# orchidas/DiffGFDN

Measured on AMD Instinct MI355X. Metric: RIR-frames/sec, higher is better.
Workload: dtype f32

## Files before the change

### diffgfdn_amd/_lib.py

```python
import ctypes
import os
from ctypes import c_char_p, c_double, c_float, c_int, c_size_t, c_void_p

_HERE = os.path.dirname(os.path.abspath(__file__))
LIB_PATH = os.path.join(_HERE, "lib", "libdiffgfdn_hip.so")
ABI_VERSION = 8

_P = c_void_p

SIGNATURES = {
    "gfdn_abi_version": (c_int, []),
    "gfdn_zprep": (c_int, [_P, c_int, _P, _P, _P]),
    "gfdn_ortho_fwd": (c_int, [_P, c_int, c_int, _P, _P, _P]),
    "gfdn_ortho_bwd": (c_int, [_P, c_int, c_int, _P, _P, _P, _P, _P]),
    "gfdn_coupled_feedback_fwd": (c_int, [_P, _P, c_int, c_int, c_int, _P, _P, _P]),
    "gfdn_coupled_feedback_bwd": (c_int, [_P, _P, c_int, c_int, c_int, _P, _P, _P, _P]),
    "gfdn_solve_fwd": (c_int, [_P, _P, c_int, c_int, c_int, _P, _P, _P, _P, c_int, _P, _P]),
    "gfdn_solve_bwd_work_bytes": (c_size_t, [c_int, c_int]),
    "gfdn_solve_bwd": (c_int, [_P, _P, c_int, c_int, c_int, _P, _P, _P, _P, c_int, _P, _P, _P, _P, _P, _P, _P]),
    "gfdn_solve_precise_fwd": (c_int, [_P, _P, c_int, c_int, c_int, _P, _P, _P, _P, c_int, _P, _P]),
    "gfdn_solve_precise_bwd": (c_int, [_P, _P, c_int, c_int, c_int, _P, _P, _P, _P, c_int, _P, _P, _P, _P, _P, _P, _P]),
    "gfdn_solve_absorb_fwd": (c_int, [_P, _P, c_int, c_int, c_int, _P, _P, _P, _P, _P, c_int, _P, _P]),
    "gfdn_solve_absorb_bwd": (c_int, [_P, _P, c_int, c_int, c_int, _P, _P, _P, _P, _P, c_int, _P, _P, _P, _P, _P, _P, _P]),
    "gfdn_solve_phi_fwd": (c_int, [_P, _P, c_int, c_int, c_int, _P, _P, _P, _P, _P, _P, _P]),
    "gfdn_solve_phi_bwd_work_bytes": (c_size_t, [c_int, c_int]),
    "gfdn_solve_phi_bwd": (c_int, [_P, _P, c_int, c_int, c_int, _P, _P, _P, _P, _P, _P, _P, _P, _P, _P, _P, _P, _P]),
    "gfdn_solve_phi_absorb_fwd": (c_int, [_P, _P, c_int, c_int, c_int, _P, _P, _P, _P, _P, _P, _P, _P]),
    "gfdn_solve_phi_absorb_bwd": (c_int, [_P, _P, c_int, c_int, c_int, _P, _P, _P, _P, _P, _P, _P, _P, _P, _P, _P, _P, _P,
                                          _P]),
    "gfdn_svf_coefficients": (c_int, [_P, _P, ctypes.c_double, c_int, c_int, _P, _P, _P]),
    "gfdn_sos_response": (c_int, [_P, c_int, c_int, _P, c_int, _P, _P]),
    "gfdn_sos_compose_fwd": (c_int, [_P, c_int, c_int, c_int, _P, c_int, _P, _P, c_int, _P, _P]),
    "gfdn_sos_compose_bwd_chunks": (c_int, [c_int, c_int, _P, _P]),
    "gfdn_sos_compose_bwd": (c_int, [_P, c_int, c_int, c_int, _P, c_int, _P, _P, _P, _P, _P]),
    "gfdn_compose_fwd": (c_int, [_P, c_int, c_int, c_int, _P, _P, c_int, _P, c_int, _P, _P, _P, c_int, _P, _P]),
    "gfdn_compose_bwd_work_bytes": (c_size_t, [c_int, c_int, c_int, c_int]),
    "gfdn_compose_bwd": (c_int, [_P, c_int, c_int, c_int, _P, _P, c_int, _P, _P, c_int, _P, _P, _P, _P, _P]),
    "gfdn_compose_banded_fwd": (c_int, [_P, c_int, c_int, c_int, c_int, _P, _P, c_int, _P, c_int, _P, _P, c_int, _P, c_int, _P, _P]),
    "gfdn_compose_banded_bwd_work_bytes": (c_size_t, [c_int, c_int, c_int, c_int, c_int]),
    "gfdn_compose_banded_bwd": (c_int, [_P, c_int, c_int, c_int, c_int, _P, _P, c_int, _P, c_int, _P, c_int, _P, _P, _P, _P, _P]),
    "gfdn_compose_sh_fwd": (c_int, [_P, c_int, c_int, c_int, _P, _P, c_int, _P, _P, _P]),
    "gfdn_compose_sh_bwd_work_bytes": (c_size_t, [c_int, c_int, c_int]),
    "gfdn_compose_sh_bwd": (c_int, [_P, c_int, c_int, c_int, _P, _P, c_int, _P, _P, _P, _P, _P, _P, _P]),
    "gfdn_spectral_stats_work_bytes": (c_size_t, [c_int, c_int]),
    "gfdn_spectral_stats": (c_int, [_P, c_int, c_int, c_int, c_float, _P, _P, _P, _P, _P]),
    "gfdn_colorless_terms": (c_int, [_P, c_int, _P, c_int, c_float, c_float, c_float, _P, _P, _P]),
    "gfdn_colorless_terms_banded": (c_int, [_P, c_int, c_int, _P, c_int, c_float, c_float, c_float, _P, _P, _P]),
    "gfdn_weighted_sums_banded": (c_int, [_P, c_int, _P, _P, c_float, _P, c_float, c_int, c_int, _P, _P]),
    "gfdn_mlp_gains_banded_fwd": (c_int, [_P, _P, _P, _P, c_int, c_int, c_int, c_int, c_int, c_int, c_float, c_float, _P, _P, _P, _P]),
    "gfdn_mlp_gains_banded_bwd": (c_int, [_P, _P, _P, _P, c_int, c_int, c_int, c_int, c_int, c_int, c_float, c_float, _P, _P, _P, _P, _P, _P, _P]),
    "gfdn_mlp_gains_banded_bwd_parts": (c_int, [_P, _P, _P, _P, c_int, c_int, c_int, c_int, c_int, c_int, c_float, c_float, _P, _P, _P, _P, c_int, _P, _P, _P]),
    "gfdn_mlp_gains_banded_bwd_parts_scaled": (c_int, [_P, _P, _P, _P, c_int, c_int, c_int, c_int, c_int, c_int, c_float, c_float,
                                                       _P, _P, _P, _P, c_int, _P, _P, _P, _P]),
    "gfdn_tf_gain_chunks": (c_int, [c_int]),
    "gfdn_mlp_bwd_takes_parts": (c_int, [c_int, c_int, c_int, c_int, c_int]),
    "gfdn_mlp_bands_sizes": (c_int, [c_int, c_int, c_int, _P, _P, c_int, _P]),
    "gfdn_mlp_gains_bands_fwd": (c_int, [_P, _P, _P, _P, c_int, c_int, c_int, _P, _P, c_int, c_float, c_float, _P, _P, _P, _P]),
    "gfdn_mlp_gains_bands_bwd": (c_int, [_P, _P, _P, _P, c_int, c_int, c_int, _P, _P, c_int, c_float, c_float, _P, _P, _P, _P,
                                         c_int, _P, _P, _P, _P]),
    "gfdn_subfdn_normalize_work_bytes": (c_size_t, [c_int]),
    "gfdn_subfdn_normalize": (c_int, [_P, _P, c_int, c_int, c_int, _P, _P, _P, _P, _P, _P, _P]),
    "gfdn_subfdn_colorless_work_bytes": (c_size_t, [c_int, c_int]),
    "gfdn_subfdn_colorless_fwd": (c_int, [_P, _P, c_int, c_int, c_int, _P, _P, _P, _P, c_int, _P, _P, _P, _P, _P]),
    "gfdn_spectral_stats_binmajor": (c_int, [_P, c_int, c_int, _P, c_int, c_float, _P, _P, _P, _P]),
    "gfdn_subfdn_colorless_bwd": (c_int, [_P, _P, c_int, c_int, c_int, _P, _P, _P, _P, _P, _P, _P, _P, _P, _P, _P, _P]),
    "gfdn_tf_coefs_fwd": (c_int, [_P, _P, _P, _P, c_int, c_int, _P, _P]),
    "gfdn_tf_coefs_fwd2": (c_int, [_P, _P, _P, _P, _P, _P, _P, _P, c_int, c_int, _P]),
    "gfdn_tf_ortho_coefs": (c_int, [_P, _P, _P, _P, c_int, c_int, _P, _P, _P, _P, _P]),
    "gfdn_tf_coefs_bwd": (c_int, [_P, _P, _P, _P, _P, _P, _P, _P, c_int, c_int, _P, _P, _P, _P, _P]),
    "gfdn_tf_param_grads": (c_int, [_P, _P, _P, c_int, _P, _P, _P, _P, _P, c_int, c_int, _P, _P, _P, _P, _P, _P, _P]),
    "gfdn_tf_rows_sum": (c_int, [_P, c_int, c_int, _P, _P]),
    "gfdn_tf_parts": (c_int, [c_int, c_int]),
    "gfdn_tf_work_bytes": (c_size_t, [c_int]),
    "gfdn_tf_gpart_bytes": (c_size_t, [c_int]),
    "gfdn_tf_eval": (c_int, [_P, _P, c_int, c_int, c_int, _P, _P, _P, _P, _P]),
    "gfdn_tf_energy": (c_int, [_P, _P, c_int, c_int, c_int, _P, _P, _P, _P, _P, _P, _P, c_int, c_double, _P]),
    "gfdn_tf_energy_gains": (c_int, [_P, _P, c_int, c_int, c_int, _P, _P, _P, _P, _P, _P, _P, c_int, c_double, _P, _P, c_int, c_int,
                                     _P]),
    "gfdn_tf_colorless": (c_int, [_P, _P, c_int, c_int, c_int, _P, _P, _P, c_int, c_float, _P, _P, _P, c_double, _P]),
    "gfdn_tf_compose_fwd": (c_int, [_P, _P, c_int, c_int, c_int, c_int, _P, _P, _P, _P, c_int, _P, c_int, _P, _P, c_int, _P, c_int, _P, _P,
                                    _P]),
    "gfdn_tf_compose_parts": (c_int, [c_int]),
    "gfdn_tf_compose_bwd_work_bytes": (c_size_t, [c_int, c_int, c_int]),
    "gfdn_tf_compose_bwd": (c_int, [_P, _P, c_int, c_int, c_int, c_int, _P, _P, _P, _P, _P, c_int, _P, c_int, _P, c_int, _P, _P,
                                    c_int, _P]),
    "gfdn_tf_tail": (c_int, [_P, _P, _P, c_int, _P, _P, _P, _P, c_int, c_int, _P, _P, _P, _P, _P, _P, _P, _P, _P, _P, _P, _P,
                             _P, c_int, c_int, c_int, c_float, c_float, c_float, _P, _P, _P, _P, _P]),
    "gfdn_irfft_odd_pairs_bwd_tslots3": (c_int, [_P, c_int, _P, _P, _P, c_int, c_int, _P, c_int, _P, _P]),
    "gfdn_irfft_odd_pairs_fwd_scaled": (c_int, [_P, c_int, _P, c_int, c_int, _P, _P, c_int, _P, c_int, _P]),
    "gfdn_edc_lin_one_max_len": (c_int, []),
    "gfdn_edc_lin_one": (c_int, [_P, c_int, _P, _P, c_int, _P, c_int, c_int, c_int, c_int, c_int, _P, _P, c_int, _P, _P,
                                 c_int, c_float, c_float, _P, _P, c_int, _P, c_int, c_int, _P]),
    "gfdn_lin_merge_slots": (c_int, [_P, _P, _P, c_int, c_int, c_int, _P, _P, c_int, _P]),
    "gfdn_f64_fft_work_bytes": (c_size_t, [c_int, c_int]),
    "gfdn_irfft_odd_f64_length": (c_int, [c_int]),
    "gfdn_rfft_pow2_f64": (c_int, [_P, c_int, c_int, c_int, c_int, _P, c_int, _P, _P]),
    "gfdn_irfft_odd_f64_plan": (c_int, [c_int, _P, _P, _P]),
    "gfdn_irfft_odd_f64": (c_int, [_P, c_int, _P, c_int, c_int, _P, _P, _P, c_int, _P, _P]),
    "gfdn_lin_gamma_win": (c_int, [_P, c_int, _P, c_int, c_int, c_int, c_int, c_int, c_int, _P, _P, _P, c_int, _P, _P, c_int,
                                   _P]),
    "gfdn_tf_gain_grad_work_bytes": (c_size_t, [c_int, c_int, c_int, c_int]),
    "gfdn_tf_gain_grad": (c_int, [c_int, c_int, c_int, c_int, _P, _P, c_int, _P, c_int, _P, _P, _P]),
    "gfdn_tf8_coefs": (c_int, [_P, _P, _P, _P, _P, _P, _P, _P, c_int, c_int, _P]),
    "gfdn_tf8_parts": (c_int, [c_int]),
    "gfdn_tf8_part_bytes": (c_size_t, [c_int, c_int]),
    "gfdn_tf8_energy": (c_int, [_P, c_int, c_int, c_int, _P, _P, _P, _P, _P, _P, _P, c_double, _P]),
    "gfdn_tf8_tsave": (c_int, [_P, c_int, c_int, c_int, c_int, _P, _P, _P, _P, _P, _P, _P, c_int, _P, _P, _P, _P]),
    "gfdn_tf8_colorless": (c_int, [_P, c_int, c_int, c_int, _P, _P, _P, _P, c_int, c_float, _P, _P, _P, c_double, _P]),
    "gfdn_tf8_compose_bwd": (c_int, [_P, c_int, c_int, c_int, c_int, _P, _P, _P, _P, _P, c_int, _P, c_int, _P, c_int, _P,
                                     _P, _P, _P]),
    "gfdn_tf8_param_grads_work_bytes": (c_size_t, [c_int]),
    "gfdn_tf8_param_grads": (c_int, [_P, _P, _P, c_int, _P, _P, _P, c_int, _P, _P, c_int, c_int, _P, _P, _P, _P, _P, _P, _P,
                                     _P]),
    "gfdn_tfp_parts": (c_int, []),
    "gfdn_tfp_forward": (c_int, [c_int, c_int, c_int, c_int, _P, _P, _P, c_int, _P, _P, c_int, _P, _P]),
    "gfdn_tfp_energy": (c_int, [_P, _P, c_int, c_int, c_int, c_int, _P, _P, _P, _P, _P, _P, _P, c_int, c_int, _P]),
    "gfdn_tfp_colorless": (c_int, [_P, _P, c_int, c_int, c_int, c_int, _P, _P, c_int, c_float, c_int, _P, _P, c_int, _P, _P, _P,
                                   _P, _P]),
    "gfdn_tfp_compose_bwd": (c_int, [c_int, c_int, c_int, c_int, _P, c_int, _P, _P, c_int, _P, c_int, _P, _P, _P, c_int, c_int,
                                     _P, c_int, _P, c_int, _P, _P, _P]),
    "gfdn_tf8_tail": (c_int, [_P, _P, _P, c_int, _P, _P, c_int, _P, _P, c_int, c_int, _P, _P, _P, _P, _P, _P, _P, _P, _P, _P, _P,
                              _P, _P, _P, c_int, c_int, c_int, c_float, c_float, c_float, _P, _P, _P, _P]),
    "gfdn_tf9_coefs": (c_int, [_P, _P, _P, c_int, c_int, _P, _P]),
    "gfdn_tf9_rec_grads_work_bytes": (c_size_t, [c_int]),
    "gfdn_tf9_rec_grads": (c_int, [_P, _P, _P, _P, _P, c_int, c_int, _P, _P, _P, _P, _P]),
    "gfdn_tfp_ratio_fwd": (c_int, [_P, _P, c_int, c_int, c_int, _P, _P, _P]),
    "gfdn_tfp_ratio_bwd": (c_int, [c_int, c_int, c_int, c_int, _P, _P, c_int, _P, _P, c_int, _P, c_int, _P, c_int, _P, _P, _P]),
    "gfdn_ortho_bwd_add": (c_int, [_P, c_int, c_int, _P, _P, _P, _P, _P, _P]),
    "gfdn_exp_contract_mfma": (c_int, [_P, c_int, _P, _P, c_int, _P, _P]),
    "gfdn_weighted_sums": (c_int, [_P, c_int, _P, _P, c_float, _P, c_float, c_int, _P, _P]),
    "gfdn_normalize_io": (c_int, [_P, _P, _P, c_int, c_int, _P]),
    "gfdn_bluestein_table_bytes": (c_size_t, [c_int]),
    "gfdn_bluestein_table_init": (c_int, [c_int, _P]),
    "gfdn_bluestein_work_bytes": (c_size_t, [c_int, c_int]),
    "gfdn_irfft_odd_fwd": (c_int, [_P, c_int, _P, c_int, c_int, _P, c_int, _P, _P]),
    "gfdn_irfft_odd_bwd": (c_int, [_P, c_int, _P, _P, c_int, c_int, _P, c_int, _P, _P]),
    "gfdn_irfft_odd_slot_order": (c_int, [c_int, _P, _P]),
    "gfdn_irfft_odd_slots_fwd": (c_int, [_P, c_int, _P, c_int, c_int, _P, c_int, _P, _P]),
    "gfdn_irfft_odd_slots_bwd": (c_int, [_P, c_int, _P, _P, c_int, c_int, _P, c_int, _P, _P]),
    "gfdn_irfft_odd_pairs_fwd": (c_int, [_P, c_int, _P, c_int, c_int, _P, c_int, _P, _P]),
    "gfdn_irfft_odd_pairs_compose_fwd": (c_int, [_P, c_int, _P, c_int, _P, _P, c_int, _P, _P, c_int, c_int, c_int, c_int, _P,
                                                 _P, c_int, _P, c_int, _P]),
    "gfdn_irfft_odd_pairs_bwd": (c_int, [_P, c_int, _P, _P, c_int, c_int, _P, c_int, _P, _P]),
    "gfdn_irfft_odd_pairs_gains_parts": (c_int, [c_int]),
    "gfdn_irfft_odd_pairs_gains_bwd": (c_int, [_P, c_int, _P, _P, c_int, c_int, _P, c_int, _P, c_int, _P, c_int, c_int, c_int, _P,
                                               _P, c_int, _P]),
    "gfdn_stft_power_pairs": (c_int, [_P, c_int, c_int, c_int, c_int, _P, _P, _P]),
    "gfdn_stft_power_pairs_bwd": (c_int, [_P, c_int, c_int, c_int, c_int, _P, _P, _P, _P]),
    "gfdn_stft_power_pairs_bwd_phase": (c_int, [_P, c_int, c_int, c_int, c_int, _P, _P, _P, c_int, _P]),
    "gfdn_edc_loss_pairs": (c_int, [_P, c_int, c_int, c_int, c_int, _P, _P, _P, c_float, c_float, _P, _P, _P, _P]),
    "gfdn_irfft_odd_stages": (c_int, [_P, c_int, _P, _P, c_int, c_int, _P, c_int, _P, c_int, c_int, c_int, _P]),
    "gfdn_irfft_pow2_work_bytes": (c_size_t, [c_int, c_int]),
    "gfdn_irfft_pow2_fwd": (c_int, [c_int, _P, c_int, c_int, _P, c_int, _P, _P]),
    "gfdn_irfft_pow2_fwd_band": (c_int, [c_int, _P, c_int, c_int, c_int, _P, c_int, c_int, _P, _P]),
    "gfdn_irfft_pow2_bwd": (c_int, [c_int, _P, c_int, c_int, _P, c_int, _P, _P]),
    "gfdn_rownorm_fwd": (c_int, [_P, c_int, c_int, c_float, _P, _P]),
    "gfdn_rownorm_bwd": (c_int, [_P, c_int, c_int, c_float, _P, _P, _P]),
    "gfdn_irfft_pow2_bwd_window": (c_int, [c_int, _P, c_int, c_int, c_int, c_int, _P, c_int, _P, _P]),
    "gfdn_edc_mixed_work_bytes": (c_size_t, [c_int, c_int, c_int]),
    "gfdn_edc_loss_model_mixed": (c_int, [_P, c_int, c_int, c_int, _P, c_int, c_int, c_int, _P, c_int, _P, c_int, _P,
                                          c_float, c_float, _P, _P, _P, _P]),
    "gfdn_group_sums_fwd": (c_int, [_P, c_int, c_int, c_int, _P, _P, _P]),
    "gfdn_group_sums_bwd": (c_int, [_P, c_int, c_int, c_int, _P, _P, _P, _P, _P, _P]),
    "gfdn_dirlin_tiles": (c_int, [c_int]),
    "gfdn_dirlin_line_tiles": (c_int, [c_int]),
    "gfdn_dirlin_lines_fwd": (c_int, [_P, c_int, c_int, _P, _P, _P, c_int, _P]),
    "gfdn_dirlin_lines_bwd": (c_int, [_P, c_int, c_int, _P, _P, _P, c_int, _P, _P, _P, _P]),
    "gfdn_dirlin_combine": (c_int, [_P, c_int, c_int, c_int, _P, c_int, c_int, c_int, _P, c_int, _P]),
    "gfdn_dirlin_gamma_dots": (c_int, [_P, c_int, c_int, _P, c_int, c_int, _P, c_int, c_int, c_int, _P, c_int, _P, _P, _P]),
    "gfdn_edc_loss_model_mixed_stages": (c_int, [_P, c_int, c_int, c_int, _P, c_int, c_int, c_int, _P, c_int, _P, c_int, _P,
                                                 c_float, c_float, _P, _P, _P, c_int, _P]),
    "gfdn_rfft_pow2": (c_int, [c_int, _P, c_int, c_int, c_int, _P, c_int, _P, _P]),
    "gfdn_sh_to_directional": (c_int, [_P, c_int, c_int, c_int, c_int, _P, _P, c_int, _P]),
    "gfdn_stft_nframes": (c_int, [c_int, c_int]),
    "gfdn_stft_power": (c_int, [_P, c_int, c_int, c_int, c_int, _P, _P, _P]),
    "gfdn_stft_power_bwd": (c_int, [_P, c_int, c_int, c_int, c_int, _P, _P, _P]),
    "gfdn_edr_work_bytes": (c_size_t, [c_int, c_int]),
    "gfdn_edr_target": (c_int, [_P, c_int, c_int, c_int, _P, _P, _P]),
    "gfdn_edr_loss": (c_int, [_P, _P, _P, _P, _P, c_int, c_int, c_int, c_float, c_int, _P, _P, _P]),
    "gfdn_edc_work_bytes": (c_size_t, [c_int]),
    "gfdn_edc_target": (c_int, [_P, c_int, c_int, c_int, c_int, _P, _P, _P]),
    "gfdn_mlp_param_count": (c_size_t, [c_int, c_int, c_int, c_int]),
    "gfdn_mlp_bwd_work_bytes": (c_size_t, [c_int, c_int, c_int, c_int, c_int]),
    "gfdn_mlp_gains_fwd": (c_int, [_P, _P, _P, _P, c_int, c_int, c_int, c_int, c_int, c_float, c_float, _P, _P, _P, _P]),
    "gfdn_mlp_gains_bwd": (c_int, [_P, _P, _P, _P, c_int, c_int, c_int, c_int, c_int, c_float, c_float, _P, _P, _P, _P, _P, _P, _P]),
    "gfdn_pick_rows": (c_int, [_P, _P, _P, c_int, _P]),
    "gfdn_adam_step": (c_int, [_P, _P, _P, _P, _P, _P, _P, c_int, c_float, c_float, c_float, _P]),
    "gfdn_adam_step_counted": (c_int, [_P, _P, _P, _P, _P, _P, _P, c_int, c_float, c_float, c_float, _P, _P]),
    "gfdn_adam_step_mirrored": (c_int, [_P, _P, _P, _P, _P, _P, _P, _P, c_int, c_float, c_float, c_float, _P, _P]),
    "gfdn_edc_loss": (c_int, [_P, c_int, c_int, c_int, c_int, _P, _P, _P, c_float, c_float, _P, _P, _P, _P]),
    "gfdn_edc_loss_model": (c_int, [_P, c_int, c_int, c_int, c_int, _P, c_int, _P, c_int, _P, c_float, c_float, _P, _P, _P, _P]),
    "gfdn_draw_mask": (c_int, [ctypes.c_ulonglong, _P, c_int, c_float, _P, _P]),
    "gfdn_lin_gain_chunks": (c_int, [c_int]),
    "gfdn_lin_combine_fwd": (c_int, [_P, c_int, _P, _P, c_int, c_int, _P, c_int, c_int, c_int, c_int, _P, c_int, c_int, _P]),
    "gfdn_lin_gamma": (c_int, [_P, _P, c_int, c_int, _P, c_int, c_int, c_int, c_int, _P, c_int, c_int, _P, _P, c_int, _P]),
    "gfdn_lin_gamma_dots_tiles": (c_int, [c_int]),
    "gfdn_lin_gamma_dots": (c_int, [_P, c_int, _P, c_int, c_int, c_int, c_int, _P, c_int, _P, c_int, _P, _P, c_int, _P, c_int,
                                    c_int, c_int, _P, _P, _P]),
    "gfdn_stft_pairs_spectrum": (c_int, [_P, c_int, c_int, c_int, c_int, _P, c_int, _P]),
    "gfdn_stft_pairs_spectrum_bwd": (c_int, [_P, c_int, c_int, c_int, _P, _P, c_int, c_int, c_int, _P, _P]),
    "gfdn_edr_lin_parts": (c_int, [c_int]),
    "gfdn_edr_lin_loss": (c_int, [_P, _P, _P, _P, c_int, c_int, c_int, _P, _P, c_int, c_int, c_float, c_int, _P, _P, _P, c_int,
                                  c_int, c_int, _P]),
    "gfdn_edr_lin_gsum": (c_int, [_P, _P, _P, _P, c_int, c_int, c_int, _P, c_int, c_int, _P, _P]),
    "gfdn_edr_lin_loss_gsum": (c_int, [_P, _P, _P, _P, c_int, c_int, c_int, _P, _P, c_int, c_int, c_float, _P, c_int, _P,
                                       c_int, c_int, _P, c_int, c_int, _P]),
    "gfdn_edr_lin_band_parts": (c_int, [c_int]),
    "gfdn_edc_loss_pairs_lin": (c_int, [_P, c_int, _P, _P, c_int, _P, c_int, c_int, c_int, c_int, c_int, c_int, _P, _P, c_int,
                                        _P, _P, c_int, c_float, c_float, _P, _P, c_int, _P, _P, _P]),
    "gfdn_irfft_odd_time_slots": (c_int, [c_int, _P]),
    "gfdn_irfft_odd_pairs_bwd_tslots": (c_int, [_P, c_int, _P, c_int, c_int, _P, c_int, _P, _P]),
    "gfdn_lin_gain_dots": (c_int, [_P, _P, c_int, c_int, _P, c_int, c_int, c_int, c_int, c_int, c_int, _P, c_int, _P]),
    "gfdn_edc_loss_banded": (c_int, [_P, c_int, c_int, c_int, c_int, _P, _P, c_int, _P, _P, c_int, c_int, c_float, c_float,
                                     _P, _P, _P, _P]),
    "gfdn_edc_loss_pairs_banded": (c_int, [_P, c_int, c_int, c_int, c_int, _P, _P, c_int, _P, _P, c_int, c_int, c_float,
                                           c_float, _P, _P, _P, _P]),
    "gfdn_draw_mask_banded": (c_int, [ctypes.c_ulonglong, _P, _P, c_int, c_int, c_int, c_float, _P, _P]),
    "gfdn_render_mix": (c_int, [_P, c_int, _P, _P, _P, c_int, c_int, c_int, c_int, _P, c_int, _P]),
}

_lib = None


def load():
    global _lib
    if _lib is not None:
        return _lib
    if not os.path.exists(LIB_PATH):
        raise RuntimeError(
            f"diffgfdn_amd: HIP library not built ({LIB_PATH}); run `make -C diffgfdn_amd/csrc` "
            "or `python -c 'import __graft_entry__ as g; g.build()'`. There is no CPU fallback.")
    import torch
    lib = ctypes.CDLL(LIB_PATH)
    for name, (res, args) in SIGNATURES.items():
        fn = getattr(lib, name)
        fn.restype = res
        fn.argtypes = args
    ver = lib.gfdn_abi_version()
# ... 11 lines not shown
```

### diffgfdn_amd/bankstep.py

```python
import contextlib
from typing import Dict, NamedTuple, Optional

import torch

from . import hip_ops as ops
from .functional import FrequencyGrid
from .losses import shard_loss_scales


_Plan = NamedTuple('_Plan', [
    ('nb', int), ('G', int), ('n', int), ('K', int), ('Ku', int), ('Btot', int), ('Bper', int), ('win', int), ('start', int),
    ('length', int),
    ('order', Optional[tuple]), ('sot', Optional[torch.Tensor]), ('tfp', Optional[tuple]),
    ('item_len', Optional[torch.Tensor]), ('band_len', Optional[torch.Tensor]),
    ('train', bool), ('normalize_first', bool), ('opt_step', bool), ('reduced', bool), ('piped', bool),
    ('big', bool), ('late', bool), ('late8', bool),
    ('lin', bool), ('spec', bool), ('pairs', bool), ('fold', bool),
    ('gfold', bool), ('parts_in_mlp', bool), ('net_first', bool), ('edc_one', bool), ('late_colorless', bool),
    ('use_tail', bool), ('use_tail8', bool), ('keep_records', bool)])


class _Step:
    scale = Hg = Ts = Dinv8 = ework = Xsub = rgain0 = rgain = xhat = rstd = H = Tq = tau = eye = xd = None
    ev_ts = ev_gam = gH = gsig = gsig_b = g_edc = gam_edr = parts = grg = None
# ... 73 lines not shown
            Q, QQ, cs = self._records()
            q, qq = ops.ortho_fwd(bank._blocks().detach(), True, True)
            Q.copy_(q)
            QQ.copy_(qq)
            cs.copy_(bank.output_gains.data.view(-1))
            self._rec_valid, self._rec_versions = True, self._versions()
            return
        ops.tf_ortho_coefs(bank._blocks().detach(), bank.inv_gamma, bank.input_gains.data.view(-1),
                           bank.output_gains.data.view(-1), out=self._records())
        self._rec_valid, self._rec_versions = True, self._versions()

    def ensure_records(self):
        if self._rec is not None and not self.records_ok():
            self.prime_records()

    linear_transforms = True
    spectral_edr = True
    edc_one_launch = True
    scale_late = True
    fused_tail = True
    transform_polys = True
    edr_one_launch = True
    edr_receiver_runs = 0

    def _edr_runs(self, nbands: int, B: int) -> int:
        if self.edr_receiver_runs > 0:
            return min(self.edr_receiver_runs, B)
        return 2 if B >= 4 else 1
    tiled_spectra = True

    def _eye_rows(self, nb: int, G: int, device) -> torch.Tensor:
        key = (nb, G, str(device))
        if getattr(self, '_eye_cache', None) is None or self._eye_cache[0] != key:
            self._eye_cache = (key, torch.eye(G, dtype=torch.float32, device=device).repeat(nb, 1).contiguous())
        return self._eye_cache[1]

    def _plan(self, data: Dict, maskw, how, reduced: bool, piped: bool) -> "_Plan":
        tr = self.tr
        normalize_first, train, opt_step = how
        bank, nb = tr.net, tr.num_bands
        G, n = bank.num_groups, bank.num_delay_lines_per_group
        z, rows = data['z_values'], data['row_index']
        Btot = rows.numel()
        if Btot % nb:
            raise ValueError("the batch must hold the same number of receivers for every band")
        Bper, K, win = Btot // nb, z.shape[-1], tr.stft_win
        side2 = tr._stream('_side2') is not None
        gridK = FrequencyGrid.of(z)
        order = ops.irfft_slot_order(K, z.device) if (tr.use_slot_order and 'dataset' in data) else None
        lin = (self.linear_transforms and not piped and ops.lin_supported(Bper, G)
               and hasattr(data.get('dataset'), 'direct_time'))
        start, length = tr._decay_window(K)
        item_len, band_len = tr._item_windows(K, Bper, z.device)
        if item_len is not None and (maskw is None or maskw.ndim != 2):
            raise ValueError("bands with different EDC windows: pass the (bands, window) weight rows of "
                             "BandBankTrainer._band_mask_rows as maskw")
        pairs = order is not None and tr.use_pairs and win == 4096
        big = n > 4
        if big and (gridK.logr is not None):
            raise NotImplementedError("blocks of more than four lines: the explicit step takes grids on the unit circle "
                                      "(set BandBankTrainer.use_fused = False to step this bank through the per-bin "
                                      "elimination kernels under autograd)")
        tail_ok = self.fused_tail and train and opt_step and not reduced and not piped and side2
        use_tail = tail_ok and not big
        late = self.scale_late and lin and order is not None and normalize_first and not big and side2
        tfp = None
        if big and self.transform_polys and lin and order is not None and gridK.rfft_nfft and side2 and normalize_first:
            T_seq = ops.tfp_plan(bank.delays, n, gridK.rfft_nfft)
            sob = ops.tfp_slot_of_bin(K, z.device)
            if T_seq is not None and sob is not None:
                tfp = (gridK.rfft_nfft, sob, T_seq)
        late8 = tfp is not None
        use_tail8 = tail_ok and late8
        spec = (lin and self.spectral_edr and pairs and ops.spec_supported(Bper, G)
                and hasattr(data['dataset'], 'direct_stft'))
        Hh, n_hidden = bank._mlp_cfg[0], bank._mlp_cfg[1]
        parts_in_mlp = ops.mlp_bwd_takes_parts(bank._freq_pi.numel(), Hh, n_hidden, G, Bper)
        if piped and (not train or reduced or not opt_step or not side2):
            raise ValueError("a pipelined step is a single-process training step with its optimiser update")
        if big:
            keep_records = use_tail8 and self.records_ok()
        else:
            keep_records = self.records_ok() and (use_tail or not train)
        return _Plan(
            nb=nb, G=G, n=n, K=K, Ku=(K + 1) // 2 if K % 2 == 1 else K, Btot=Btot, Bper=Bper, win=win, start=start,
            length=length, order=order, tfp=tfp, item_len=item_len, band_len=band_len,
            sot=ops.irfft_slot_of_time(K, z.device) if (lin and train and order is not None) else None,
            train=train, normalize_first=normalize_first, opt_step=opt_step, reduced=reduced, piped=piped, big=big, lin=lin,
            pairs=pairs, spec=spec, late=late, late8=late8, use_tail=use_tail, use_tail8=use_tail8, keep_records=keep_records,
            parts_in_mlp=parts_in_mlp,
            gfold=(late or late8) and not piped and spec and train and parts_in_mlp,
            fold=pairs and K == 65537 and Bper % 2 == 0 and G <= 4 and not lin,
            late_colorless=big or spec,
            edc_one=self.edc_one_launch and ops.edc_lin_one_supported(length, G),
            net_first=bool(getattr(bank, 'mixed_networks', False)))

    def _begin(self, p: "_Plan", data: Dict, maskw, inv: float, calls: Dict) -> "_Step":
        tr = self.tr
        bank, z = tr.net, data['z_values']
        if p.lin:
            zu, direct = (data['dataset'].slot_grid(*p.order) if p.order is not None else z[:p.Ku]), None
        elif p.order is not None:
            zu, direct = data['dataset'].slot_ordered(*p.order)
        else:
            zu, direct = z[:p.Ku], data['target_early_response'][:, :p.Ku]
        return _Step(
            **calls, data=data, rows=data['row_index'], maskw=maskw, inv=inv, keep=self._keep,
            main=torch.cuda.current_stream(), side=tr._stream('_side'), side2=tr._stream('_side2'),
            M=bank._blocks().detach(), b=bank.input_gains.data.view(-1), c=bank.output_gains.data.view(-1),
            delays=bank.delays, ig=bank.inv_gamma, w=bank.output_scalars_w.detach(), gridK=FrequencyGrid.of(z), zu=zu,
            direct=direct, inv_world=shard_loss_scales(tr.world_size, 1, 1.0)['colorless'],
            T_edr=data['edr_target'][1], sum_abs=data['edr_target'][2], T_edc=data['edc_target'][1],
            ev={k: torch.cuda.Event() for k in ('start', 'g', 'h', 'mlp', 'mask', 'norm', 'x', 'edc', 'side', 'grg', 'mlpb')})

    def _gain_network(self, st: "_Step", out=None):
        bank = self.tr.net
        Hh, n_hidden, _, lo, hi = bank._mlp_cfg
        return ops.mlp_gains_fwd(st.data['norm_listener_position'], bank._freq_pi, st.w, Hh, n_hidden, bank.num_groups, lo, hi,
                                 st.rows, self.tr.num_bands, out=out)

    def _wait_gains(self, st: "_Step"):
        if st.pipe is None:
            st.main.wait_event(st.ev['mlp'])
        elif st.pipe.ready is not None:
            st.main.wait_event(st.pipe.ready)

    def _records_head(self, p: "_Plan", st: "_Step"):
        ev, keep, late_any = st.ev, st.keep, p.late or p.late8
        if not late_any:
            ev['start'].record()
        st.c_head = st.c
        if p.big:
            if p.keep_records:
                st.Q, st.QQ, st.c_head = self._records()
            else:
                st.Q, st.QQ = ops.ortho_fwd(st.M, True, True)
                if p.late8:
                    st.c_head = st.c.detach().clone()
                    keep.append(st.c_head)
            st.coef, st.coef_sub = ops.tf8_coefs(st.QQ, st.ig, st.b, st.c, A1=st.M)
        else:
            if not p.keep_records:
                ops.tf_ortho_coefs(st.M, st.ig, st.b, st.c, out=self._records())
            st.Q, st.QQ, st.coef, st.coef_sub = self._records()
        self._rec_valid = False
        if late_any:
            ev['start'].record()
        st.gridU = FrequencyGrid.of(st.zu)
        st.filt = self.tr._filter_on(p.Ku, p.order)
        gridK, gridU = st.gridK, st.gridU
        if p.late:
            st.Hg, st.Ts = ops.tf_compose_fwd(gridU.turns, gridU.logr, st.coef, st.delays, p.n,
                                              self._eye_rows(p.nb, p.G, st.rows.device), None, None, st.filt, None, p.nb,
                                              save_T=True, want_H=True)
        if p.late8:
            st.Ts, _, st.Hg, st.Dinv8 = ops.tf8_tsave(gridK.turns[:p.Ku], st.coef, st.delays, p.n, st.c_head, None, p.nb, p.G,
                                                      quad=False, filt=st.filt, want_H=True, hslot=p.tfp[1])
            keep.append(st.Dinv8)
        if p.normalize_first and not late_any:
            if p.big:
                _, st.scale = ops.tf8_energy(gridK.turns, st.coef_sub, st.delays, p.n, st.b, st.c, dturn=gridK.dturn)
            else:
                _, st.scale = ops.tf_energy(gridK.turns, gridK.logr, st.coef_sub, st.delays, p.n, st.b, st.c,
                                            want_energy=False, dturn=gridK.dturn)
        if not late_any:
            ev['norm'].record()

    def _side_head(self, p: "_Plan", st: "_Step"):
        ev, keep, gridK, pipe = st.ev, st.keep, st.gridK, st.pipe
        energy = (gridK.turns, gridK.logr, st.coef_sub, st.delays, p.n, st.b, st.c)
        with st.on_side2():
            if pipe is None or pipe.first:
                torch.cuda.current_stream().wait_event(ev['start'])
            if p.gfold and p.big:
                st.rgain0, st.xhat, st.rstd = self._gain_network(st)
                keep.append(st.rgain0)
            if p.late:
                if p.gfold:
                    if p.net_first:
                        st.rgain0, st.xhat, st.rstd = self._gain_network(st)
                    st.ework = ops.tf_energy(*energy, phase=1, dturn=gridK.dturn)
                    if not p.net_first:
                        st.rgain0, st.xhat, st.rstd = self._gain_network(st)
                    keep.append(st.rgain0)
                    _, st.scale, st.rgain = ops.tf_energy(*energy, want_energy=False, work=st.ework, phase=2,
                                                          dturn=gridK.dturn, gains=st.rgain0, G=p.G)
                else:
                    _, st.scale = ops.tf_energy(*energy, want_energy=False, dturn=gridK.dturn)
                ev['norm'].record()
            elif p.late8:
                nblk8 = p.nb * p.G
                st.Xsub = ops.tfp_forward(st.coef_sub, st.delays, st.c, p.n, p.tfp[0], p.tfp[2])
                if p.gfold:
                    _, st.scale, st.rgain = ops.tfp_energy(st.Xsub[:nblk8], st.Xsub[nblk8:], p.n, st.b, st.c, gains=st.rgain0,
                                                           G=p.G)
                else:
                    _, st.scale = ops.tfp_energy(st.Xsub[:nblk8], st.Xsub[nblk8:], p.n, st.b, st.c)
                ev['norm'].record()
                keep.append(st.Xsub)
            if p.gfold:
                ev['mlp'].record()
            elif pipe is None:
                st.rgain, st.xhat, st.rstd = self._gain_network(st)
                ev['mlp'].record()
            else:
                st.rgain, st.xhat, st.rstd = pipe.cur
            if st.mask_draw is not None:
                st.mask_draw()
            ev['mask'].record()

    def _group_signals(self, p: "_Plan", st: "_Step"):
        gridU, K = st.gridU, p.K
        st.eye = self._eye_rows(p.nb, p.G, st.rows.device)
        st.xd = st.data['dataset'].direct_time(self.tr.subband_filter_freq_resp, K)
        if p.late8:
            pass
        elif p.big:
            st.Ts, _, st.Hg, st.Dinv8 = ops.tf8_tsave(gridU.turns, st.coef, st.delays, p.n, st.c, st.scale, p.nb, p.G,
                                                      quad=False, filt=st.filt, want_H=True)
            st.keep.append(st.Dinv8)
            st.ev_ts = torch.cuda.Event()
            st.ev_ts.record()
        elif not p.late:
            st.Hg, st.Ts = ops.tf_compose_fwd(gridU.turns, gridU.logr, st.coef, st.delays, p.n, st.eye, st.scale, None,
                                              st.filt, None, p.nb, save_T=True, want_H=True)
        if p.gfold:
            st.tau = ops.irfft_odd_fwd(st.Hg, K, slots=True, pairs=True)
        elif p.late or p.late8:
            st.tau = ops.irfft_odd_fwd(st.Hg, K, slots=True, pairs=True, oscale=st.scale,
                                       before_last=lambda: st.main.wait_event(st.ev['norm']))
        else:
            st.tau = ops.irfft_odd_fwd(st.Hg, K, slots=p.order is not None, pairs=p.order is not None)
        st.H = st.Hg
        st.keep.extend((st.tau, st.xd))

    def _stored_output_stage(self, p: "_Plan", st: "_Step"):
        gridU = st.gridU
        if not p.fold:
            self._wait_gains(st)
        if p.big:
            st.Ts, Tq8 = ops.tf8_tsave(gridU.turns, st.coef, st.delays, p.n, st.c, st.scale, p.nb, p.G, quad=True)
            st.ev_ts = torch.cuda.Event()
            st.ev_ts.record()
            if p.fold:
                st.H = Tq8
            else:
                Hs = torch.einsum('qbg,qgk->qbk', st.rgain.reshape(p.nb, p.Bper, p.G).to(torch.complex64),
                                  st.Ts.reshape(p.nb, p.G, -1))
                Hs = Hs + st.direct[st.rows].reshape(p.nb, p.Bper, -1)[..., :st.Ts.shape[1]]
                if st.filt is not None:
                    Hs = Hs * st.filt.reshape(p.nb, 1, -1)
                st.H = Hs.reshape(p.Btot, -1).contiguous()
        else:
            st.H, st.Ts = ops.tf_compose_fwd(gridU.turns, gridU.logr, st.coef, st.delays, p.n, st.rgain, st.scale, st.direct,
                                             st.filt, st.rows, p.nb, save_T=True, want_H=not p.fold)
        if p.fold:
            st.Tq, st.H = st.H, None

    def _colorless(self, p: "_Plan", st: "_Step"):
        cfg, gridK, weight = self.tr.config, st.gridK, self.tr.config.spectral_loss_weight * st.inv_world
        with st.on_side2():
            if not p.late and not p.late8:
                torch.cuda.current_stream().wait_event(st.ev['norm'])
            if p.late8:
                nblk8 = p.nb * p.G
                grec_sub, loss_g = ops.tfp_colorless(st.Xsub[:nblk8], st.Xsub[nblk8:], p.tfp[0], p.n, st.delays, st.scale,
                                                     cfg.use_asym_spectral_loss, weight, T=p.tfp[2])
            elif p.big:
                torch.cuda.current_stream().wait_event(st.ev_ts)
                grec_sub, loss_g = ops.tf8_colorless(gridK.turns, st.coef_sub, st.delays, p.n, st.c, st.scale,
                                                     cfg.use_asym_spectral_loss, weight, dturn=gridK.dturn)
            else:
                grec_sub, loss_g = ops.tf_colorless(gridK.turns, gridK.logr, st.coef_sub, st.delays, p.n, st.scale,
                                                    cfg.use_asym_spectral_loss, weight, dturn=gridK.dturn)
            st.out3, st.gQ = ops.colorless_terms(loss_g, st.Q, cfg.spectral_loss_weight, cfg.sparsity_loss_weight,
                                                 st.inv_world, want_grad=p.train, nbands=p.nb)
            st.ev['side'].record()
        st.grec_sub = grec_sub
        st.keep.extend((grec_sub, loss_g, st.out3, st.gQ))

    def _receiver_signals(self, p: "_Plan", st: "_Step") -> torch.Tensor:
        if p.lin:
            self._wait_gains(st)
            return ops.lin_combine_fwd(st.xd, st.rows, st.tau, st.rgain, p.nb, p.K, p.order is not None, p.pairs)
        if p.fold:
            self._wait_gains(st)
            x2, h0 = ops.irfft_odd_pairs_compose_fwd(st.direct, st.rows, st.Tq, st.rgain, st.filt, p.K, p.nb)
            st.keep.extend((h0, st.Tq))
            return x2
        if p.pairs:
            return ops.irfft_odd_fwd(st.H, p.K, slots=True, pairs=True)
        return ops.irfft_odd_fwd(st.H, p.K, slots=p.order is not None)

    def _decay_stored(self, p: "_Plan", st: "_Step"):
        cfg, keep, ev, main = self.tr.config, st.keep, st.ev, st.main
        K, Btot, win, train = p.K, p.Btot, p.win, p.train
        x = self._receiver_signals(p, st)
        ev['x'].record()
        if p.pairs:
            P = ops.stft_power_pairs(x, Btot, win)
            g_edr = None
        else:
            g_edr = torch.empty_like(x) if train else None
            P = ops.stft_power(x, win, zero_buf=g_edr)
        with st.on_side2():
            torch.cuda.current_stream().wait_event(ev['x'])
            if p.pairs:
                li_edc, g_edc = ops.edc_loss_pairs(x, Btot, p.start, p.length, st.T_edc, st.maskw, st.inv, cfg.edc_loss_weight,
                                                   train, rows=st.rows, item_len=p.item_len, items_per_band=p.Bper)
            else:
                li_edc, g_edc = ops.edc_loss(x, p.start, p.length, st.T_edc, st.maskw, st.inv, cfg.edc_loss_weight, train,
                                             rows=st.rows, item_len=p.item_len, items_per_band=p.Bper)
            ev['edc'].record()
        li_edr = ops.edr_loss(P, st.T_edr, st.sum_abs, None, cfg.edr_loss_weight, train, rows=st.rows, defer=True)
        keep.extend((x, P, g_edr, li_edc, g_edc, li_edr))
        gH = None
        if train:
            if p.pairs:
                g = ops.stft_power_pairs_bwd(x, Btot, win, P, phase=0)
                main.wait_event(ev['edc'])
                ops.stft_power_pairs_bwd(x, Btot, win, P, base=g_edc, out=g, phase=1)
                ev['g'].record()
                gH = (g, None) if p.lin else ops.irfft_odd_pairs_bwd(g, K, Btot)
                keep.append(g)
            else:
                g_edr = ops.stft_power_bwd(x, win, P, g_edr)
                main.wait_event(ev['edc'])
                ev['g'].record()
                if p.lin:
                    gH = (g_edc, g_edr)
                else:
                    gH = ops.irfft_odd_bwd(g_edc, K, (K + 1) // 2 if p.order is not None else st.H.shape[1], g_edr,
                                           slots=p.order is not None)
            keep.append(gH)
        else:
            main.wait_event(ev['edc'])
            ev['g'].record()
        st.li_edr, st.li_edc, st.gH = li_edr, li_edc, gH

    def _decay_spec(self, p: "_Plan", st: "_Step"):
        tr, cfg, keep, ev = self.tr, self.tr.config, st.keep, st.ev
        nb, G, K, win, train = p.nb, p.G, p.K, p.win, p.train
        rows, rgain, tau, ds, tiled = st.rows, st.rgain, st.tau, st.data['dataset'], self.tiled_spectra
        Sd = ds.direct_stft(tr.subband_filter_freq_resp, K, win, tiled=tiled)
        T_edr = ds.edr_target_tiled() if tiled else st.T_edr
        ev['x'].record()
        nch = 1 if p.edc_one else ops.lin_gamma_dots_tiles(K)
        parts = None
        if train:
            parts = torch.empty((p.Btot * G, nch + ops.edr_lin_parts(win // 2 + 1, fused=self.edr_one_launch)),
                                dtype=torch.float32, device=rows.device)
        Stau = ops.stft_pairs_spectrum(tau, nb * G, win, tiled=tiled)
        with st.on_side2():
            torch.cuda.current_stream().wait_event(ev['x'])
            edc_args = (st.xd, rows, tau, rgain, nb, K, p.start, p.length, st.T_edc, st.maskw, st.inv, cfg.edc_loss_weight,
                        train)
            if p.edc_one:
                li_edc, g_edc = ops.edc_lin_one(*edc_args, trows=rows, item_len=p.item_len, dots=parts, col=0)
                if train:
                    g_edc = (g_edc, ops.lin_gamma_win(g_edc, rgain, nb, K, p.start, p.length, band_win_len=p.band_len))
            else:
                li_edc, g_edc = ops.edc_loss_pairs_lin(*edc_args, trows=rows, item_len=p.item_len, fill_outside=False)
            ev['edc'].record()
        self._wait_gains(st)
        gP = Gs = None
        if train and self.edr_one_launch:
            li_edr, Gs = ops.edr_lin_loss_gsum(Sd, rows, Stau, rgain, nb, T_edr, st.sum_abs, cfg.edr_loss_weight, dots=parts,
                                               col0=nch, tiled=tiled, nsplit=self._edr_runs(nb, p.Bper))
        else:
            li_edr, gP = ops.edr_lin_loss(Sd, rows, Stau, rgain, nb, T_edr, st.sum_abs, cfg.edr_loss_weight, train,
                                          dots=parts, col0=nch, tiled=tiled)
        if not train:
            ev['g'].record()
        keep.extend((Sd, Stau, li_edc, g_edc, li_edr, gP, parts))
        st.li_edr, st.li_edc, st.gH = li_edr, li_edc, None
        if not train:
            st.main.wait_event(ev['edc'])
            return
        if Gs is None:
            Gs = ops.edr_lin_gsum(Sd, rows, Stau, rgain, nb, gP)
        gam_edr = ops.stft_pairs_spectrum_bwd(Gs, K, nb * G, win, tiled=tiled, split_parity=True)
        keep.extend((Gs, gam_edr))
        st.g_edc, st.gam_edr, st.parts = g_edc, gam_edr, parts

    def _report(self, p: "_Plan", st: "_Step"):
        cfg = self.tr.config
        s_ = ops.weighted_sums(st.li_edr, cfg.edr_loss_weight, st.li_edc, cfg.edc_loss_weight, st.sum_abs, st.rows, p.nb)
        st.sums, st.total = s_, ((s_[:, 0] + st.out3[:, 0]) if p.nb > 1 else (s_[0] + st.out3[0]))

    def _adjoint_signals(self, p: "_Plan", st: "_Step"):
        K, nb, keep = p.K, p.nb, st.keep
        if not p.lin:
            st.gH_rec, st.rg_rec = st.gH, st.rgain
            return
        tau_pairs = p.order is not None
        if p.spec:
            st.gsig, st.gsig_b = st.g_edc, None
            st.main.wait_event(st.ev['edc'])
            ge_a, ge_b = st.gam_edr if isinstance(st.gam_edr, tuple) else (st.gam_edr, None)
            if isinstance(st.gsig, tuple):
                gam = ops.lin_merge_slots(st.gsig[1], ge_a, ge_b, p.sot)
            else:
                gam = ops.lin_gamma_dots(st.gsig, st.rgain, nb, K, st.tau, st.parts, p.start, p.length, base=ge_a,
                                         slot_of_time=p.sot, band_win_len=p.band_len, base_b=ge_b)
            st.ev_gam = torch.cuda.Event()
            st.ev_gam.record()
        else:
            st.gsig, st.gsig_b = st.gH
            gam = ops.lin_gamma(st.gsig, st.rgain, nb, K, p.pairs, tau_pairs, gxb=st.gsig_b, slot_of_time=p.sot)
        if tau_pairs:
            gHg = ops.irfft_odd_pairs_bwd(gam, K, nb * p.G, tslots=p.sot is not None)
        else:
            gHg = ops.irfft_odd_bwd(gam, K, p.Ku, None, slots=False)
        keep.extend((gam, gHg, st.eye))
        st.gH_rec, st.rg_rec = gHg, st.eye

    def _records_pass(self, p: "_Plan", st: "_Step"):
        gridU = st.gridU
        if p.late8:
            st.grec = ops.tfp_compose_bwd(p.tfp[0], p.nb, p.G, p.n, st.delays, p.Ku, p.tfp[1], st.gH_rec, st.filt, st.Ts,
                                          st.Dinv8, tscale=st.scale, gain_fold=p.gfold, T=p.tfp[2])
        elif p.big:
            st.grec = ops.tf8_compose_bwd(gridU.turns, st.coef, st.delays, p.n, st.c, st.scale, st.rg_rec, st.gH_rec, st.filt,
                                          p.nb, saved=(st.Ts, st.Dinv8) if p.lin else None)
        else:
            st.grec = ops.tf_compose_bwd(gridU.turns, gridU.logr, st.coef, st.delays, p.n, st.rg_rec, st.gH_rec, st.Ts, st.filt,
                                         p.nb, partial=True, tscale=st.scale if p.late else None,
                                         gain_fold=p.gfold and p.late)

    def _side_backward(self, p: "_Plan", st: "_Step"):
        tr, ev, pipe = self.tr, st.ev, st.pipe
        bank, opt, nb, G = tr.net, tr.optimizer, p.nb, p.G
        Hh, n_hidden, _, lo, hi = bank._mlp_cfg
        with st.on_side2():
            cur = torch.cuda.current_stream()
            cur.wait_event(st.ev_gam if p.spec else ev['g'])
            self._report(p, st)
            if st.allreduce is not None:
                slots = opt.extra.view(3, nb)
                torch.stack((st.sums.reshape(nb, 3)[:, 1], st.sums.reshape(nb, 3)[:, 2], st.out3.reshape(nb, 3)[:, 0]),
                            out=slots)
            grg = None
            if p.lin:
                if p.spec:
                    cur.wait_event(st.ev_gam)
                    ggp = st.parts
                else:
                    ggp = ops.lin_gain_dots(st.gsig, st.tau, nb, p.Btot, G, p.K, p.pairs, p.order is not None, gxb=st.gsig_b)
                if not p.parts_in_mlp:
                    grg, ggp = ops.tf_rows_sum(ggp).view(p.Btot, G), None
            else:
                cur.wait_event(ev['grg'])
                if p.parts_in_mlp:
                    ggp = ops.tf_gain_grad(st.Ts, st.gH, G, st.filt, nb, partial=True)
                else:
                    grg, ggp = ops.tf_gain_grad(st.Ts, st.gH, G, st.filt, nb), None
            ops.mlp_gains_bwd(st.data['norm_listener_position'], bank._freq_pi, st.w, Hh, n_hidden, G, lo, hi,
                              st.rgain0 if p.gfold else st.rgain, st.xhat, st.rstd, grg, st.rows, nb, out=self.g_w,
                              ggains_parts=ggp, colscale=st.scale if p.gfold else None)
            st.keep.append(ggp)
            if pipe is not None:
                opt.step_range(*self.w_range, second=True)
                if st.tail is not None:
                    st.tail()
                self._gain_network(st, out=pipe.nxt)
                pipe.ready_next = torch.cuda.Event()
                pipe.ready_next.record()
            else:
                if p.use_tail or p.use_tail8:
                    opt.step_range(*self.w_range, second=True)
                ev['mlpb'].record()
                if st.tail is not None:
                    st.tail()
        st.grg = grg

    def _parameter_tail(self, p: "_Plan", st: "_Step"):
        tr, opt = self.tr, self.tr.optimizer
        rec = (st.QQ, st.ig, st.grec, st.grec_sub, st.b, st.c, st.M, st.gQ, st.Q, self.g_b, self.g_c)
        if p.use_tail8:
            ops.tf8_tail(*rec, self.g_M, opt, *self._off, *self._records())
        elif p.big:
            ops.tf8_param_grads(st.QQ, st.ig, st.grec, st.b, st.c, st.M, A1=st.M, part1=st.grec_sub, gQ=st.gQ, Q=st.Q,
                                gb=self.g_b, gc=self.g_c, gM=self.g_M)
        elif p.use_tail:
            ops.tf_tail(*rec, self.g_M.view(-1), opt, *self._off, *self._records())
        else:
            ops.tf_param_grads(st.QQ, st.ig, st.grec, st.b, st.c, st.M, A1=st.M, grec1=st.grec_sub, gQ=st.gQ, Q=st.Q,
                               gb=self.g_b, gc=self.g_c, gM=self.g_M)
        st.keep.extend((st.grg, st.grec))
        if p.piped:
            opt.step_range(0, self.w_range[0], second=False)
            torch.autograd.graph.increment_version(opt._params)
            return
        opt._packed = True
        if p.use_tail or p.use_tail8:
            opt._packed = False
            torch.autograd.graph.increment_version(opt._params)
            self._rec_valid, self._rec_versions = True, self._versions()
        elif p.opt_step and not p.reduced and st.side2 is not None:
            ev_pg = torch.cuda.Event()
            ev_pg.record()
            with st.on_side2():
                torch.cuda.current_stream().wait_event(ev_pg)
                self.finish(None)
        else:
            st.main.wait_event(st.ev['mlpb'])
            if p.opt_step:
                red = self.finish(st.allreduce)
                if red is not None:
                    st.sums, st.total = red

    def _losses(self, p: "_Plan", st: "_Step") -> Dict:
        col = (lambda t, i: t[:, i]) if p.nb > 1 else (lambda t, i: t[i])
        return {'edc_loss': col(st.sums, 2), 'edr_loss': col(st.sums, 1), 'spectral_loss': col(st.out3, 1),
                'sparsity_loss': col(st.out3, 2), '_total': st.total}

    def _end(self, p: "_Plan", st: "_Step") -> Dict:
        keep, pipe = st.keep, st.pipe
        keep.extend((st.sums, st.total))
        losses = self._losses(p, st)
        if pipe is None or pipe.last:
            for s_ in (st.side, st.side2):
                if s_ is not None:
                    st.main.wait_stream(s_)
        if pipe is not None:
            self._keep_prev = [] if pipe.last else list(keep)
            keep.clear()
            pipe.advance()
            return losses
        keep.clear()
        if not p.big and not p.train and not p.normalize_first:
            self._rec_valid, self._rec_versions = True, self._versions()
        return losses

    @torch.no_grad()
    def run(self, data: Dict, maskw: Optional[torch.Tensor], inv: float, normalize_first: bool, train: bool,
            allreduce=None, opt_step: bool = True, mask_draw=None, tail=None, pipe=None) -> Dict:
        p = self._plan(data, maskw, (normalize_first, train, opt_step), allreduce is not None, pipe is not None)
        st = self._begin(p, data, maskw, inv, dict(allreduce=allreduce, mask_draw=mask_draw, tail=tail, pipe=pipe))
        self._records_head(p, st)
        self._side_head(p, st)
        if p.lin:
            self._group_signals(p, st)
        else:
            self._stored_output_stage(p, st)
        st.keep.extend((st.coef_sub, st.ework, st.Q, st.QQ, st.coef, st.rgain, st.xhat, st.rstd, st.scale, st.H, st.Ts))
        if not p.late_colorless:
            self._colorless(p, st)
        st.ev['h'].record()
        if p.spec:
            self._decay_spec(p, st)
        else:
            self._decay_stored(p, st)
        if p.late_colorless:
            self._colorless(p, st)
        if not train:
            with st.on_side2():
                torch.cuda.current_stream().wait_event(st.ev['g'])
                self._report(p, st)
            return self._end(p, st)
        if (p.use_tail or p.use_tail8) and not torch.cuda.is_current_stream_capturing():
            self.tr.optimizer.sync_lr()
        st.ev['grg'].record()
        self._adjoint_signals(p, st)
        self._records_pass(p, st)
        self._side_backward(p, st)
        st.main.wait_event(st.ev['side'])
        self._parameter_tail(p, st)
        return self._end(p, st)

    def finish(self, allreduce):
        tr = self.tr
        nb = tr.num_bands
        red = None
        if allreduce is not None:
            allreduce()
        tr.optimizer.step()
        if allreduce is not None:
            slots = tr.optimizer.extra.view(3, nb)
            total = slots.sum(dim=0)
            sums = torch.stack((total, slots[0], slots[1]), dim=1)
# ... 33 lines not shown
```

### diffgfdn_amd/csrc/blocktf.hip

```cpp
#include "common.h"
#include "ortho_dev.h"

#define TF_MAXBLK 64
#define TF_REC 32
#define TF_MAXG 4
#define TF_MAX_PARTS 2048

__device__ __forceinline__ float2 tf_zpow(const double* __restrict__ turns, const double* __restrict__ logr,
                                          int k, float m) {
  double t = (double)m * turns[k];
  t -= rint(t);
  float s, c;
  sincospif(2.0f * (float)t, &s, &c);
  if (logr) {
    const float mag = (float)exp((double)m * logr[k]);
    c *= mag;
    s *= mag;
  }
  return make_float2(c, s);
}

__device__ __forceinline__ void tf_subsets(float2 (&e)[16]) {
  e[3] = cmul(e[1], e[2]);
  e[5] = cmul(e[1], e[4]);
// ... 676 lines not shown
extern "C" int gfdn_tf_energy_gains(const double* turns, const double* logr, int K, int nblk, int nper, const float* coef,
                                    const float* delays, float* b, float* c, float* energy, float* scale, void* work,
                                    int phase, double dturn, const float* gains, float* gains_scaled, int Bper, int G,
                                    void* stream) {
  if (!gains || !gains_scaled || Bper <= 0 || G <= 0 || nblk % G || !(phase & 2)) return GFDN_E_BADARG;
  return tf_energy_run(turns, logr, K, nblk, nper, coef, delays, b, c, energy, scale, work, phase, dturn, gains, gains_scaled, Bper,
                       G, stream);
}
static int tf_energy_run(const double* turns, const double* logr, int K, int nblk, int nper, const float* coef,
                         const float* delays, float* b, float* c, float* energy, float* scale, void* work, int phase,
                         double dturn, const float* gains, float* gains_scaled, int Bper, int G, void* stream) {
  int rc = tf_args_ok(turns, K, nblk, nper, coef, delays);
  if (rc) return rc;
  if (!work || (!b) != (!c) || !(phase & 3)) return GFDN_E_BADARG;
  TfArgs a{turns, logr, K, nblk, nper, coef, delays, nullptr};
  const int nparts = tf_parts_host(K, nblk);
  hipStream_t s = (hipStream_t)stream;
  if (phase & 1) {
    if (dturn != 0.0 && !logr)
      hipLaunchKernelGGL(k_tf_energy_runs, dim3(nparts), dim3(256), 0, s, a, dturn, (float*)work, tf_items(nblk));
    else
      hipLaunchKernelGGL(k_tf_energy, dim3(nparts), dim3(256), 0, s, a, (float*)work, tf_items(nblk));
    GFDN_LAUNCH_CHECK();
  }
  if (phase & 2) {
    hipLaunchKernelGGL(k_tf_energy_finish, dim3(nblk), dim3(256), 0, s, (const float*)work, nparts, K, nper, b, c,
                       energy, scale, gains, gains_scaled, Bper, G);
    GFDN_LAUNCH_CHECK();
  }
  return 0;
}

template <bool RUNS>
__global__ __launch_bounds__(256) void k_tf_colorless(TfArgs a, double dturn, int asym, float gscale,
                                                      float* __restrict__ gpart, int items) {
  extern __shared__ float tf_acc[];
  const int nblk = a.nblk;
  const bool live = (int)threadIdx.x < items;
  const int blk = live ? threadIdx.x % nblk : 0;
  const int krow = threadIdx.x / nblk, rows = items / nblk;
  float P[16], Q[16], m[4];
  tf_load(a.coef, a.delays, blk, a.nper, P, Q, m);
  const float sc = a.scale ? a.scale[blk] : 1.0f;
  const float invK = 1.0f / (float)a.K;
  float2 r0, r1, r2, r3;
  if (RUNS) {
    r0 = tf_rot(dturn, m[0]);
    r1 = tf_rot(dturn, m[1]);
    r2 = tf_rot(dturn, m[2]);
    r3 = tf_rot(dturn, m[3]);
  }
  float aP[16], aQ[16];
#pragma unroll
  for (int S = 0; S < 16; ++S) aP[S] = aQ[S] = 0.f;
  constexpr int RUN = RUNS ? TF_RUN : 1;
  const int nruns = (a.K + RUN - 1) / RUN;
#pragma unroll 1
  for (int run = blockIdx.x * rows + krow; live && run < nruns; run += gridDim.x * rows) {
    const int k0 = run * RUN;
    float2 e[16];
    e[1] = tf_zpow(a.turns, RUNS ? nullptr : a.logr, k0, m[0]);
    e[2] = tf_zpow(a.turns, RUNS ? nullptr : a.logr, k0, m[1]);
    e[4] = tf_zpow(a.turns, RUNS ? nullptr : a.logr, k0, m[2]);
    e[8] = tf_zpow(a.turns, RUNS ? nullptr : a.logr, k0, m[3]);
#pragma unroll 1
    for (int j = 0; j < RUN; ++j) {
      if (k0 + j >= a.K) break;
      float2 num, den;
      tf_subsets(e);
      tf_numden(P, Q, e, num, den);
      const float2 dinv = cinv(den);
      const float2 s = cscale(cmul(num, dinv), sc);
      const float mag = sqrtf(s.x * s.x + s.y * s.y);
      const float d = mag - 1.0f, d2 = d * d;
      const bool four = asym && (d > 1.0f);
      aP[15] += (four ? d2 * d2 : d2) * invK;
      const float dl = four ? 4.0f * d2 * d : 2.0f * d;
      const float f = (mag > 0.f) ? gscale * invK * dl / mag : 0.f;
      const float2 gs = make_float2(f * s.x, f * s.y);
      const float2 u = cmulc(gs, dinv);
      const float2 v = cmulc(u, s);
      aP[0] += u.x;
      aQ[0] -= v.x;
#pragma unroll
      for (int S = 1; S < 16; ++S) {
        if (S < 15) aP[S] += u.x * e[S].x + u.y * e[S].y;
        aQ[S] -= v.x * e[S].x + v.y * e[S].y;
      }
      if (RUNS) {
        e[1] = cmul(e[1], r0);
        e[2] = cmul(e[2], r1);
        e[4] = cmul(e[4], r2);
        e[8] = cmul(e[8], r3);
      }
    }
  }
  if (live) {
#pragma unroll
    for (int S = 0; S < 16; ++S) {
      tf_acc[threadIdx.x * 33 + S] = aP[S];
      tf_acc[threadIdx.x * 33 + 16 + S] = aQ[S];
    }
  }
  __syncthreads();
  for (int o = threadIdx.x; o < nblk * TF_REC; o += 256) {
    const int bq = o >> 5, e = o & 31;
    float sum = 0.f;
    for (int t = bq; t < items; t += nblk) sum += tf_acc[t * 33 + e];
    gpart[(size_t)o * gridDim.x + blockIdx.x] = sum;
  }
}

extern "C" size_t gfdn_tf_gpart_bytes(int nblk) {
  return (size_t)TF_MAX_PARTS * (nblk > 0 ? nblk : 1) * TF_REC * sizeof(float);
}

extern "C" int gfdn_tf_colorless(const double* turns, const double* logr, int K, int nblk, int nper,
                                 const float* coef, const float* delays, const float* scale, int asym,
                                 float gscale, float* grec, float* loss, void* work, double dturn, void* stream) {
  int rc = tf_args_ok(turns, K, nblk, nper, coef, delays);
  if (rc) return rc;
  if (!grec || !work) return GFDN_E_BADARG;
  TfArgs a{turns, logr, K, nblk, nper, coef, delays, scale};
  const int nparts = tf_parts_host(K, nblk), items = tf_items(nblk);
  hipStream_t s = (hipStream_t)stream;
  if (dturn != 0.0 && !logr)
    hipLaunchKernelGGL(k_tf_colorless<true>, dim3(nparts), dim3(256), (size_t)items * 33 * sizeof(float), s, a, dturn,
                       asym, gscale, (float*)work, items);
  else
    hipLaunchKernelGGL(k_tf_colorless<false>, dim3(nparts), dim3(256), (size_t)items * 33 * sizeof(float), s, a, 0.0,
                       asym, gscale, (float*)work, items);
  GFDN_LAUNCH_CHECK();
  const int rows = nblk * TF_REC;
  hipLaunchKernelGGL(k_tf_rows_sum, dim3((rows + 3) / 4), dim3(256), 0, s, (const float*)work, nparts, rows, grec, rows,
                     (float*)nullptr, loss);
  GFDN_LAUNCH_CHECK();
  return 0;
}

struct TfCompose {
  const double* turns;
  const double* logr;
  int K, G, nper, B;
  const float* coef;
  const float* delays;
  const float* scale;
  const float* rgain;
  const float2* filt;
  int ldf;
  int fold;
};

#define TFC_BCH 8
__global__ __launch_bounds__(256) void k_tf_compose_fwd(TfCompose a, const float2* __restrict__ direct, int ldd,
                                                        const long long* __restrict__ drows,
                                                        float2* __restrict__ H, int ldh, float2* __restrict__ Tsave,
                                                        float2* __restrict__ Tquad) {
  __shared__ TfBlock tab[TF_MAXG];
  const int band = blockIdx.y, G = a.G, B = a.B;
  tf_stage(a.coef, a.delays, band * G, G, a.nper, tab);
  __syncthreads();
  const int k = blockIdx.x * 256 + threadIdx.x;
  if (k >= a.K) return;
  const float* rgain = a.rgain + (size_t)band * B * G;
  if (drows) drows += (size_t)band * B;
  else if (direct) direct += (size_t)band * B * ldd;
  if (H) H += (size_t)band * B * ldh;
  else direct = nullptr;
  float2 d[TFC_BCH];
#pragma unroll
  for (int bb = 0; bb < TFC_BCH; ++bb)
    d[bb] = (direct && bb < B) ? direct[(size_t)(drows ? drows[bb] : bb) * ldd + k] : make_float2(0.f, 0.f);
  float2 T[TF_MAXG];
#pragma unroll
  for (int g = 0; g < TF_MAXG; ++g) {
    T[g] = make_float2(0.f, 0.f);
    if (g < G) {
      float2 e[16], num, den;
      tf_phasors(a.turns, a.logr, k, tab[g].m, e);
      tf_numden(tab[g].P, tab[g].Q, e, num, den);
      T[g] = cmul(num, cinv(den));
      if (a.scale) T[g] = cscale(T[g], a.scale[band * G + g]);
      if (Tsave) Tsave[(size_t)(band * G + g) * a.K + k] = T[g];
    }
  }
  if (Tquad) {
    float4* q = (float4*)(Tquad + ((size_t)band * a.K + k) * 4);
    q[0] = make_float4(T[0].x, T[0].y, T[1].x, T[1].y);
    q[1] = make_float4(T[2].x, T[2].y, T[3].x, T[3].y);
  }
  if (!H) return;
  const float2 f = a.filt ? a.filt[(size_t)band * a.ldf + k] : make_float2(1.f, 0.f);
  for (int b0 = 0; b0 < B; b0 += TFC_BCH) {
    float2 dn[TFC_BCH];
#pragma unroll
    for (int bb = 0; bb < TFC_BCH; ++bb) {
      const int b = b0 + TFC_BCH + bb;
      dn[bb] = (direct && b < B) ? direct[(size_t)(drows ? drows[b] : b) * ldd + k] : make_float2(0.f, 0.f);
    }
#pragma unroll
    for (int bb = 0; bb < TFC_BCH; ++bb) {
      const int b = b0 + bb;
      if (b < B) {
        float2 h = d[bb];
#pragma unroll
        for (int g = 0; g < TF_MAXG; ++g) {
          if (g < G) {
            const float rg = rgain[b * G + g];
            h.x += rg * T[g].x;
            h.y += rg * T[g].y;
          }
        }
        if (a.filt) h = cmul(h, f);
        H[(size_t)b * ldh + k] = h;
      }
    }
#pragma unroll
    for (int bb = 0; bb < TFC_BCH; ++bb) d[bb] = dn[bb];
  }
}

static int tf_compose_ok(const double* turns, int K, int nbands, int G, int nper, int B, const float* coef,
                         const float* delays, const float* rgain) {
  if (!turns || !coef || !delays || !rgain || K <= 0 || nbands <= 0 || G <= 0 || nper <= 0 || B <= 0)
    return GFDN_E_BADARG;
  if (nper > 4 || G > TF_MAXG || nbands > 65535) return GFDN_E_UNSUPPORTED;
  return 0;
}

extern "C" int gfdn_tf_compose_fwd(const double* turns, const double* logr, int K, int nbands, int G, int nper,
                                   const float* coef, const float* delays, const float* scale,
                                   const float* rgain, int B, const float* direct, int ldd,
                                   const long long* direct_rows, const float* filt, int ldf, float* H, int ldh,
                                   float* Tsave, float* Tquad, void* stream) {
  int rc = tf_compose_ok(turns, K, nbands, G, nper, B, coef, delays, rgain);
  if (rc) return rc;
  if ((!H && !Tsave && !Tquad) || (H && ldh < K) || (direct && ldd < K) || (filt && nbands > 1 && ldf < K)) return GFDN_E_BADARG;
  TfCompose a{turns, logr, K, G, nper, B, coef, delays, scale, rgain, (const float2*)filt, ldf};
  hipLaunchKernelGGL(k_tf_compose_fwd, dim3((K + 255) / 256, nbands), dim3(256), 0, (hipStream_t)stream, a,
                     (const float2*)direct, ldd, direct ? direct_rows : nullptr, (float2*)H, ldh, (float2*)Tsave,
                     (float2*)Tquad);
  GFDN_LAUNCH_CHECK();
  return 0;
}

#define TFB_T 64
#define TFG_R 8
#define TFG_PRIO 0
__global__ __launch_bounds__(256) void k_tf_gain_grad(const float2* __restrict__ Tsave, int K, int G, int B,
                                                      const float2* __restrict__ filt, int ldf,
                                                      const float2* __restrict__ gH, int ldh,
                                                      float* __restrict__ rg_partial, int ngrp) {
  if (TFG_PRIO) __builtin_amdgcn_s_setprio(TFG_PRIO);
  __shared__ float s_red[4][TFG_R * TF_MAXG];
  const int band = blockIdx.y / ngrp, b0 = (blockIdx.y - band * ngrp) * TFG_R;
  const int nr = B - b0 < TFG_R ? B - b0 : TFG_R;
  const float2* T0 = Tsave + (size_t)band * G * K;
  const float2* g0 = gH + ((size_t)band * B + b0) * ldh;
  float acc[TFG_R][TF_MAXG];
#pragma unroll
  for (int r = 0; r < TFG_R; ++r)
#pragma unroll
    for (int g = 0; g < TF_MAXG; ++g) acc[r][g] = 0.f;
  for (int k = blockIdx.x * 256 + threadIdx.x; k < K; k += gridDim.x * 256) {
    float2 gh[TFG_R];
#pragma unroll
    for (int r = 0; r < TFG_R; ++r) gh[r] = r < nr ? g0[(size_t)r * ldh + k] : make_float2(0.f, 0.f);
    const float2 f = filt ? filt[(size_t)band * ldf + k] : make_float2(1.f, 0.f);
    float2 w[TF_MAXG];
#pragma unroll
    for (int g = 0; g < TF_MAXG; ++g) w[g] = g < G ? cmul(f, T0[(size_t)g * K + k]) : make_float2(0.f, 0.f);
#pragma unroll
    for (int r = 0; r < TFG_R; ++r)
#pragma unroll
      for (int g = 0; g < TF_MAXG; ++g) acc[r][g] += gh[r].x * w[g].x + gh[r].y * w[g].y;
  }
  const int lane = threadIdx.x & 63, wv = threadIdx.x >> 6;
#pragma unroll
  for (int r = 0; r < TFG_R; ++r)
#pragma unroll
    for (int g = 0; g < TF_MAXG; ++g) {
      const float v = wave_sum(acc[r][g]);
      if (lane == 0) s_red[wv][r * TF_MAXG + g] = v;
    }
  __syncthreads();
  if (threadIdx.x < TFG_R * TF_MAXG) {
    const int r = threadIdx.x / TF_MAXG, g = threadIdx.x % TF_MAXG;
    if (r < nr && g < G) {
      const float v = (s_red[0][threadIdx.x] + s_red[1][threadIdx.x]) + (s_red[2][threadIdx.x] + s_red[3][threadIdx.x]);
      rg_partial[((size_t)band * B * G + (size_t)(b0 + r) * G + g) * gridDim.x + blockIdx.x] = v;
    }
  }
}

#define TFR_BCH 8
__global__ __launch_bounds__(256) void k_tf_compose_bwd_rec(TfCompose a, const float2* __restrict__ Tsave,
                                                            const float2* __restrict__ gH, int ldh,
                                                            float* __restrict__ gpart) {
  __shared__ TfBlock tab[TF_MAXG];
  const int band = blockIdx.y, G = a.G, B = a.B, nparts = gridDim.x;
  tf_stage(a.coef, a.delays, band * G, G, a.nper, tab);
  __syncthreads();
  const int lane = threadIdx.x & 63, w = __builtin_amdgcn_readfirstlane(threadIdx.x >> 6);
  if (w >= G) return;
  const float* rgain = a.rgain + (size_t)band * B * G + w;
  gH += (size_t)band * B * ldh;
  const float2* Tp = Tsave + (size_t)(band * G + w) * a.K;
  float Q[16], m[4];
#pragma unroll
  for (int S = 0; S < 16; ++S) Q[S] = tab[w].Q[S];
#pragma unroll
  for (int r = 0; r < 4; ++r) m[r] = tab[w].m[r];
  float aP[16], aQ[16];
#pragma unroll
  for (int S = 0; S < 16; ++S) aP[S] = aQ[S] = 0.f;
  const float tsc = a.scale ? a.scale[band * G + w] : 1.0f;
  const float itsc = 1.0f / tsc;
  const int ntiles = (a.K + TFB_T - 1) / TFB_T;
  for (int tile = blockIdx.x; tile < ntiles; tile += nparts) {
    const int k = tile * TFB_T + lane;
    const bool live = k < a.K;
    const int kk = live ? k : a.K - 1;
    float2 acc = make_float2(0.f, 0.f);
    for (int b0 = 0; b0 < B; b0 += TFR_BCH) {
      float2 gh[TFR_BCH];
#pragma unroll
      for (int i = 0; i < TFR_BCH; ++i)
        gh[i] = (live && b0 + i < B) ? gH[(size_t)(b0 + i) * ldh + kk] : make_float2(0.f, 0.f);
#pragma unroll
      for (int i = 0; i < TFR_BCH; ++i) {
        const float rg = b0 + i < B ? rgain[(b0 + i) * G] : 0.f;
        acc.x += rg * gh[i].x;
        acc.y += rg * gh[i].y;
      }
    }
    if (a.filt) acc = cmulc(acc, a.filt[(size_t)band * a.ldf + kk]);
    float2 e[16];
    tf_phasors(a.turns, a.logr, kk, m, e);
    float2 den = make_float2(Q[0], 0.f);
#pragma unroll
    for (int S = 1; S < 16; ++S) {
      den.x += Q[S] * e[S].x;
      den.y += Q[S] * e[S].y;
    }
    float2 u = cmulc(acc, cinv(den));
    float2 v;
    if (a.fold) {
      v = cmulc(u, Tp[kk]);
      u = cscale(u, itsc);
    } else {
      v = cmulc(u, a.scale ? cscale(Tp[kk], tsc) : Tp[kk]);
    }
    aP[0] += u.x;
    aQ[0] -= v.x;
#pragma unroll
    for (int S = 1; S < 16; ++S) {
      if (S < 15) aP[S] += u.x * e[S].x + u.y * e[S].y;
      aQ[S] -= v.x * e[S].x + v.y * e[S].y;
    }
  }
  float* out = gpart + (size_t)(band * G + w) * TF_REC * nparts + blockIdx.x;
#pragma unroll
  for (int S = 0; S < 16; ++S) {
    const float p = wave_sum_full(aP[S]), q = wave_sum_full(aQ[S]);
    if (lane == 0) {
      out[(size_t)S * nparts] = p;
      out[(size_t)(16 + S) * nparts] = q;
    }
  }
}

static int tf_compose_parts_host(int K) {
  const int tiles = (K + TFB_T - 1) / TFB_T;
  int parts = (tiles + 3) / 4;
  if (parts > TF_MAX_PARTS) parts = TF_MAX_PARTS;
  return parts < 1 ? 1 : parts;
}
static int tf_gain_chunks_host(int K) {
  int c = (K + 1023) / 1024;
  if (c > 32) c = 32;
  return c < 1 ? 1 : c;
}
extern "C" int gfdn_tf_compose_parts(int K) { return K > 0 ? tf_compose_parts_host(K) : 0; }
extern "C" size_t gfdn_tf_compose_bwd_work_bytes(int K, int nbands, int G) {
  if (K <= 0 || nbands <= 0 || G <= 0) return 0;
  return (size_t)nbands * G * TF_REC * tf_compose_parts_host(K) * sizeof(float);
}
extern "C" size_t gfdn_tf_gain_grad_work_bytes(int K, int nbands, int G, int B) {
  if (K <= 0 || nbands <= 0 || G <= 0 || B <= 0) return 0;
  return (size_t)nbands * G * B * tf_gain_chunks_host(K) * sizeof(float);
}

extern "C" int gfdn_tf_gain_grad(int K, int nbands, int G, int B, const float* Tsave, const float* filt, int ldf,
                                 const float* gH, int ldh, float* grgain, void* work, void* stream) {
  if (!Tsave || !gH || !work || K <= 0 || nbands <= 0 || G <= 0 || B <= 0 || ldh < K ||
      (filt && nbands > 1 && ldf < K))
    return GFDN_E_BADARG;
  if (G > TF_MAXG || nbands * ((B + TFG_R - 1) / TFG_R) > 65535) return GFDN_E_UNSUPPORTED;
  const int nchunk = tf_gain_chunks_host(K), ngrp = (B + TFG_R - 1) / TFG_R;
  hipStream_t s = (hipStream_t)stream;
  hipLaunchKernelGGL(k_tf_gain_grad, dim3(nchunk, nbands * ngrp), dim3(256), 0, s, (const float2*)Tsave, K, G, B,
                     (const float2*)filt, ldf, (const float2*)gH, ldh, (float*)work, ngrp);
  GFDN_LAUNCH_CHECK();
  if (!grgain) return 0;
  const int nrg = nbands * B * G;
  hipLaunchKernelGGL(k_tf_rows_sum, dim3((nrg + 3) / 4), dim3(256), 0, s, (const float*)work, nchunk, nrg, grgain, nrg,
                     (float*)nullptr, (float*)nullptr);
  GFDN_LAUNCH_CHECK();
  return 0;
}
extern "C" int gfdn_tf_gain_chunks(int K) { return K > 0 ? tf_gain_chunks_host(K) : 0; }

extern "C" int gfdn_tf_compose_bwd(const double* turns, const double* logr, int K, int nbands, int G, int nper,
                                   const float* coef, const float* delays, const float* Tsave, const float* tscale,
                                   const float* rgain, int B, const float* filt, int ldf, const float* gH,
                                   int ldh, float* grec, void* work, int gain_fold, void* stream) {
  int rc = tf_compose_ok(turns, K, nbands, G, nper, B, coef, delays, rgain);
  if (rc) return rc;
  if (!Tsave || !gH || !work || ldh < K || (filt && nbands > 1 && ldf < K) || (gain_fold && !tscale)) return GFDN_E_BADARG;
  TfCompose a{turns, logr, K, G, nper, B, coef, delays, tscale, rgain, (const float2*)filt, ldf, gain_fold ? 1 : 0};
  const int nparts = tf_compose_parts_host(K);
  hipStream_t s = (hipStream_t)stream;
  hipLaunchKernelGGL(k_tf_compose_bwd_rec, dim3(nparts, nbands), dim3(256), 0, s, a, (const float2*)Tsave,
                     (const float2*)gH, ldh, (float*)work);
  GFDN_LAUNCH_CHECK();
  if (!grec) return 0;
  const int n0 = nbands * G * TF_REC;
  hipLaunchKernelGGL(k_tf_rows_sum, dim3((n0 + 3) / 4), dim3(256), 0, s, (const float*)work, nparts, n0, grec, n0,
                     (float*)nullptr, (float*)nullptr);
  GFDN_LAUNCH_CHECK();
  return 0;
}
```

### diffgfdn_amd/csrc/common.h

```cpp
#pragma once
#include <hip/hip_runtime.h>
#include <mutex>
#include <stddef.h>
#include <stdint.h>

#include "../../include/diffgfdn_hip.h"

#define GFDN_LAUNCH_CHECK()                      \
  do {                                           \
    hipError_t e__ = hipGetLastError();          \
    if (e__ != hipSuccess) return (int)e__;      \
  } while (0)

#define F32_EPS 1.1920928955078125e-07f
#define TEN_OVER_LN10 4.3429448190325175f

__device__ __forceinline__ float2 cmul(float2 a, float2 b) {
  return make_float2(a.x * b.x - a.y * b.y, a.x * b.y + a.y * b.x);
}
__device__ __forceinline__ float2 cmulc(float2 a, float2 b) {
  return make_float2(a.x * b.x + a.y * b.y, a.y * b.x - a.x * b.y);
}
__device__ __forceinline__ float2 cadd(float2 a, float2 b) { return make_float2(a.x + b.x, a.y + b.y); }
__device__ __forceinline__ float2 csub(float2 a, float2 b) { return make_float2(a.x - b.x, a.y - b.y); }
__device__ __forceinline__ float2 cinv(float2 a) {
  float d = 1.0f / (a.x * a.x + a.y * a.y);
  return make_float2(a.x * d, -a.y * d);
}
__device__ __forceinline__ float2 cconj(float2 a) { return make_float2(a.x, -a.y); }
__device__ __forceinline__ float2 cscale(float2 a, float s) { return make_float2(a.x * s, a.y * s); }

__device__ __forceinline__ float db_pow(float x) {
  float y = 10.0f * log10f(fabsf(x) + F32_EPS);
  return fmaxf(y, -200.0f);
}

__device__ __forceinline__ float adam_elem(float p, float g, float& m, float& v, float lr, float bc1, float bc2_sqrt,
                                           float b1, float b2, float eps) {
  m = __fmaf_rn(g - m, 1.0f - b1, m);
  v = __fmaf_rn(__fmul_rn(g, g), 1.0f - b2, __fmul_rn(v, b2));
  const float denom = __fadd_rn(__fdiv_rn(sqrtf(v), bc2_sqrt), eps);
  return __fsub_rn(p, __fmul_rn(__fdiv_rn(lr, bc1), __fdiv_rn(m, denom)));
}

struct TfAdam {
  float* p;
  float* m;
  float* v;
  const unsigned char* seg;
  const float* lr_seg;
  float* step_count;
  unsigned int* block_counter;
  int offM, offb, offc;
  float b1, b2, eps;
};

__device__ __forceinline__ float tf_adam_elem(const TfAdam& ad, int i, float gi, float bc1, float bc2_sqrt) {
  float mi = ad.m[i], vi = ad.v[i];
  const float pn = adam_elem(ad.p[i], gi, mi, vi, ad.lr_seg[ad.seg[i]], bc1, bc2_sqrt, ad.b1, ad.b2, ad.eps);
  ad.m[i] = mi;
  ad.v[i] = vi;
  ad.p[i] = pn;
  return pn;
}


template <int CTRL>
__device__ __forceinline__ float dpp_pair_sum(float v) {
  return v + __int_as_float(__builtin_amdgcn_update_dpp(0, __float_as_int(v), CTRL, 0xf, 0xf, false));
}
__device__ __forceinline__ float xor16_sum(float x) {
  const auto r = __builtin_amdgcn_permlane16_swap(__float_as_uint(x), __float_as_uint(x), false, false);
  return __uint_as_float(r[0]) + __uint_as_float(r[1]);
}
__device__ __forceinline__ float xor32_sum(float x) {
  const auto r = __builtin_amdgcn_permlane32_swap(__float_as_uint(x), __float_as_uint(x), false, false);
  return __uint_as_float(r[0]) + __uint_as_float(r[1]);
}
__device__ __forceinline__ float wave_sum_full(float v) {
  v = dpp_pair_sum<0x128>(v);
  v = dpp_pair_sum<0x124>(v);
  v = dpp_pair_sum<0x122>(v);
  v = dpp_pair_sum<0x121>(v);
  return xor32_sum(xor16_sum(v));
}
__device__ __forceinline__ float wave_sum(float v) {
#pragma unroll
  for (int off = 32; off >= 1; off >>= 1) v += __shfl_xor(v, off, 64);
  return v;
}

template <int CTRL>
__device__ __forceinline__ float dpp_add_shifted(float v) {
  return v + __int_as_float(__builtin_amdgcn_update_dpp(0, __float_as_int(v), CTRL, 0xf, 0xf, true));
}
__device__ __forceinline__ float readlane_f(float v, int lane) {
  return __int_as_float(__builtin_amdgcn_readlane(__float_as_int(v), lane));
}
__device__ __forceinline__ float wave_scan_incl(float v, float& total) {
  v = dpp_add_shifted<0x111>(v);
  v = dpp_add_shifted<0x112>(v);
  v = dpp_add_shifted<0x114>(v);
  v = dpp_add_shifted<0x118>(v);
  const float t0 = readlane_f(v, 15), t1 = readlane_f(v, 31), t2 = readlane_f(v, 47), t3 = readlane_f(v, 63);
  const int row = (threadIdx.x & 63) >> 4;
  const float add = (row >= 1 ? t0 : 0.f) + (row >= 2 ? t1 : 0.f) + (row >= 3 ? t2 : 0.f);
  total = ((t0 + t1) + t2) + t3;
  return v + add;
}
__device__ __forceinline__ float wave_scan_incl_rev(float v, float& total) {
  v = dpp_add_shifted<0x101>(v);
  v = dpp_add_shifted<0x102>(v);
  v = dpp_add_shifted<0x104>(v);
  v = dpp_add_shifted<0x108>(v);
  const float t0 = readlane_f(v, 0), t1 = readlane_f(v, 16), t2 = readlane_f(v, 32), t3 = readlane_f(v, 48);
  const int row = (threadIdx.x & 63) >> 4;
  const float add = (row <= 2 ? t3 : 0.f) + (row <= 1 ? t2 : 0.f) + (row <= 0 ? t1 : 0.f);
  total = ((t3 + t2) + t1) + t0;
  return v + add;
}
__device__ __forceinline__ float wave_sum_valu(float v) {
  float total;
  wave_scan_incl(v, total);
  return total;
}

__device__ __forceinline__ float block_sum(float v, float* lds ) {
  v = wave_sum(v);
  int w = threadIdx.x >> 6, nw = (blockDim.x + 63) >> 6;
  __syncthreads();
  if ((threadIdx.x & 63) == 0) lds[w] = v;
  __syncthreads();
  float s = 0.f;
  for (int i = 0; i < nw; ++i) s += lds[i];
  return s;
}

static inline int ensure_dyn_lds_ptr(const void* fn, size_t bytes) {
  if (bytes <= 48 * 1024) return 0;
  constexpr int SLOTS = 512;
  static const void* fns[SLOTS];
  static size_t granted[SLOTS];
  static int count = 0;
  static std::mutex mu;
  std::lock_guard<std::mutex> lock(mu);
  int slot = -1;
  for (int i = 0; i < count; ++i)
    if (fns[i] == fn) { slot = i; break; }
  if (slot >= 0 && bytes <= granted[slot]) return 0;
  int rc = (int)hipFuncSetAttribute(fn, hipFuncAttributeMaxDynamicSharedMemorySize, (int)bytes);
  if (rc != 0) return rc;
  if (slot < 0 && count < SLOTS) { slot = count++; fns[slot] = fn; }
  if (slot >= 0) granted[slot] = bytes;
  return 0;
}
template <typename K>
static inline int ensure_dyn_lds(K kernel, size_t bytes) {
  return ensure_dyn_lds_ptr(reinterpret_cast<const void*>(kernel), bytes);
}

static inline int ilog2(int v) {
  int l = 0;
  while ((1 << l) < v) ++l;
  return l;
}
static inline int next_pow2(int v) { return 1 << ilog2(v); }
```

### diffgfdn_amd/csrc/solve.hip

```cpp
#include "common.h"

__global__ void k_zprep(const double* __restrict__ z, int K, double* __restrict__ turns,
                        double* __restrict__ logr) {
  int k = blockIdx.x * blockDim.x + threadIdx.x;
  if (k >= K) return;
  double re = z[2 * k], im = z[2 * k + 1];
  turns[k] = atan2(im, re) * 0.15915494309189535;
  logr[k] = 0.5 * log(re * re + im * im);
}

extern "C" int gfdn_zprep(const double* z, int K, double* turns, double* logr, void* stream) {
  if (!z || !turns || !logr || K <= 0) return GFDN_E_BADARG;
  hipLaunchKernelGGL(k_zprep, dim3((K + 255) / 256), dim3(256), 0, (hipStream_t)stream, z, K,
                     turns, logr);
  GFDN_LAUNCH_CHECK();
  return 0;
}

__device__ __forceinline__ float2 zeta_pow(const double* __restrict__ turns,
                                           const double* __restrict__ logr, int k, float m,
                                           float inv_gamma) {
  double t = (double)m * turns[k];
  t -= rint(t);
  float s, c;
// ... 2205 lines not shown
  const float2 f = filt ? filt[k] : make_float2(1.f, 0.f);
  const float2* yrow = yt + threadIdx.x * NS;
  for (int bb = 0; bb < nb; ++bb) {
    const float* sb = sw + bb * N;
    for (int l = 0; l < nper; ++l) {
      float2 h = make_float2(0.f, 0.f);
      for (int g = 0; g < G; ++g) {
        const int n = g * nper + l;
        const float2 y = yrow[n];
        h.x += sb[n] * y.x;
        h.y += sb[n] * y.y;
      }
      if (filt) h = cmul(h, f);
      H[((size_t)(b0 + bb) * nper + l) * K + k] = h;
    }
  }
}

extern "C" int gfdn_compose_sh_fwd(const float* Y, int K, int G, int nper, const float* c,
                                   const float* w, int B, const float* filt, float* H,
                                   void* stream) {
  if (!Y || !c || !w || !H || K <= 0 || G <= 0 || nper <= 0 || B <= 0) return GFDN_E_BADARG;
  const int N = G * nper, NS = N + 1 + (N & 1);
  const size_t lds = (size_t)SH_TB * NS * sizeof(float2) + (size_t)SH_BCH * N * sizeof(float);
  int rc = ensure_dyn_lds(k_compose_sh_fwd, lds);
  if (rc) return rc;
  hipLaunchKernelGGL(k_compose_sh_fwd, dim3((K + SH_TB - 1) / SH_TB, (B + SH_BCH - 1) / SH_BCH), dim3(SH_TB), lds,
                     (hipStream_t)stream, (const float2*)Y, K, G, nper, c, w, B, (const float2*)filt, (float2*)H);
  GFDN_LAUNCH_CHECK();
  return 0;
}

__global__ __launch_bounds__(SH_TB) void k_compose_sh_bwd_y(const float2* __restrict__ Y, int K, int G,
                                                            int nper, const float* __restrict__ c,
                                                            const float* __restrict__ w, int B,
                                                            const float2* __restrict__ filt,
                                                            const float2* __restrict__ gH,
                                                            float2* __restrict__ gY,
                                                            float* __restrict__ gc_partial) {
  const int N = G * nper, NS = N + 1 + (N & 1);
  constexpr int NW = SH_TB / 64;
  float2* yt = compose_lds;
  float2* sgh = yt + SH_TB * NS;
  float* sw = (float*)(sgh + nper * SH_TB);
  float* sg = sw + B * N;
  int* lch = (int*)(sg + NW * N);
  const int k0 = blockIdx.x * SH_TB;
  const int nbin = K - k0 < SH_TB ? K - k0 : SH_TB;
  const size_t base = (size_t)k0 * N;
  for (int e = threadIdx.x; e < SH_TB * N; e += SH_TB) {
    const int kq = e / N, n = e - kq * N;
    yt[kq * NS + n] = e < nbin * N ? Y[base + e] : make_float2(0.f, 0.f);
  }
  for (int e = threadIdx.x; e < B * N; e += SH_TB) sw[e] = w[e];
  for (int e = threadIdx.x; e < N; e += SH_TB) lch[e] = e % nper;
  __syncthreads();
  const int k = k0 + threadIdx.x;
  const bool valid = k < K;
  const int kk = valid ? k : K - 1;
  const int lane = threadIdx.x & 63, wv = threadIdx.x >> 6;
  const float2 fc = filt ? cconj(filt[kk]) : make_float2(1.f, 0.f);
  float2* yrow = yt + threadIdx.x * NS;
  float2 acc[GFDN_MAX_SH_LINES];
#pragma unroll
  for (int n = 0; n < GFDN_MAX_SH_LINES; ++n) acc[n] = make_float2(0.f, 0.f);
  for (int b = 0; b < B; ++b) {
    const float* swb = sw + b * N;
    for (int l = 0; l < nper; ++l) {
      float2 gh = valid ? gH[((size_t)b * nper + l) * K + kk] : make_float2(0.f, 0.f);
      if (filt) gh = cmul(gh, fc);
      sgh[l * SH_TB + threadIdx.x] = gh;
    }
#pragma unroll
    for (int n = 0; n < GFDN_MAX_SH_LINES; ++n) {
      if (n < N) {
        const float2 gh = sgh[lch[n] * SH_TB + threadIdx.x];
        acc[n].x += swb[n] * gh.x;
        acc[n].y += swb[n] * gh.y;
      }
    }
  }
#pragma unroll
  for (int n = 0; n < GFDN_MAX_SH_LINES; ++n) {
    if (n < N) {
      const float2 y = yrow[n];
      const float v = wave_sum(valid ? (acc[n].x * y.x + acc[n].y * y.y) : 0.f);
      if (lane == 0) sg[wv * N + n] = v;
      yrow[n] = cscale(acc[n], c[n]);
    }
  }
  __syncthreads();
  for (int e = threadIdx.x; e < N; e += SH_TB) {
    float sum = 0.f;
#pragma unroll
    for (int q = 0; q < NW; ++q) sum += sg[q * N + e];
    gc_partial[(size_t)blockIdx.x * N + e] = sum;
  }
  for (int e = threadIdx.x; e < nbin * N; e += SH_TB) {
    const int kq = e / N, n = e - kq * N;
    gY[base + e] = yt[kq * NS + n];
  }
}

#define SH_KT 64
#define SH_KC 512
__global__ __launch_bounds__(SH_TB) void k_compose_sh_bwd_w(const float2* __restrict__ Y, int K, int G,
                                                            int nper, const float* __restrict__ c, int B,
                                                            const float2* __restrict__ filt,
                                                            const float2* __restrict__ gH,
                                                            float* __restrict__ partial) {
  const int N = G * nper;
  const int rb = SH_TB / G;
  float2* ta = compose_lds;
  float2* ty = ta + rb * (SH_KT + 1);
  const int l = blockIdx.y, b0 = blockIdx.z * rb;
  const int nb = B - b0 < rb ? B - b0 : rb;
  const int bb = threadIdx.x / G, g = threadIdx.x - bb * G;
  const bool mine = bb < nb;
  const int kbeg = blockIdx.x * SH_KC;
  float acc = 0.f;
  for (int ks = kbeg; ks < kbeg + SH_KC && ks < K; ks += SH_KT) {
    for (int e = threadIdx.x; e < rb * SH_KT; e += SH_TB) {
      const int r = e / SH_KT, kq = e - r * SH_KT;
      const int k = ks + kq;
      float2 v = make_float2(0.f, 0.f);
      if (r < nb && k < K) {
        v = gH[((size_t)(b0 + r) * nper + l) * K + k];
        if (filt) v = cmul(v, cconj(filt[k]));
      }
      ta[r * (SH_KT + 1) + kq] = v;
    }
    for (int e = threadIdx.x; e < SH_KT * G; e += SH_TB) {
      const int kq = e / G, gg = e - kq * G;
      const int k = ks + kq;
      ty[e] = k < K ? Y[(size_t)k * N + gg * nper + l] : make_float2(0.f, 0.f);
    }
    __syncthreads();
    if (mine) {
      const float2* ar = ta + bb * (SH_KT + 1);
#pragma unroll 8
      for (int kq = 0; kq < SH_KT; ++kq) {
        const float2 a = ar[kq], y = ty[kq * G + g];
        acc += a.x * y.x + a.y * y.y;
      }
    }
    __syncthreads();
  }
  if (mine) {
    const int n = g * nper + l;
    partial[((size_t)blockIdx.x * B + b0 + bb) * N + n] = acc * c[n];
  }
}

template <int NV>
__device__ __forceinline__ float wave_sums_transposed32(const float (&v)[NV]) {
  const int lane = threadIdx.x & 63;
  float a[16];
#pragma unroll
  for (int i = 0; i < 16; ++i) {
    const unsigned lo_v = __float_as_uint(i < NV ? v[i < NV ? i : 0] : 0.f);
    const unsigned hi_v = __float_as_uint(i + 16 < NV ? v[i + 16 < NV ? i + 16 : 0] : 0.f);
    const auto r = __builtin_amdgcn_permlane32_swap(lo_v, hi_v, false, false);
    a[i] = __uint_as_float(r[0]) + __uint_as_float(r[1]);
  }
#pragma unroll
  for (int i = 0; i < 8; ++i) {
    const auto r = __builtin_amdgcn_permlane16_swap(__float_as_uint(a[i]), __float_as_uint(a[i + 8]), false, false);
    a[i] = __uint_as_float(r[0]) + __uint_as_float(r[1]);
  }
  {
    const bool hi = lane & 8;
#pragma unroll
    for (int i = 0; i < 4; ++i) {
      const float s0 = dpp_pair_sum<0x128>(a[i]), s1 = dpp_pair_sum<0x128>(a[i + 4]);
      a[i] = hi ? s1 : s0;
    }
  }
  {
    const bool hi = lane & 4;
#pragma unroll
    for (int i = 0; i < 2; ++i) {
      const float s0 = dpp_pair_sum<0x141>(a[i]), s1 = dpp_pair_sum<0x141>(a[i + 2]);
      a[i] = hi ? s1 : s0;
    }
  }
  {
    const float s0 = dpp_pair_sum<0x4e>(a[0]), s1 = dpp_pair_sum<0x4e>(a[1]);
    a[0] = (lane & 2) ? s1 : s0;
  }
  return dpp_pair_sum<0xb1>(a[0]);
}

#define SHF_TB 64
template <int NPER>
__global__ __launch_bounds__(256, NPER <= 9 ? 4 : 2) void k_compose_sh_bwd_fused(const float2* __restrict__ Y, int K, int G,
                                                              const float* __restrict__ c,
                                                              const float* __restrict__ w, int B,
                                                              const float2* __restrict__ filt,
                                                              const float2* __restrict__ gH,
                                                              float2* __restrict__ gY,
                                                              float* __restrict__ partial) {
  constexpr int MAXG = NPER <= 4 ? 8 : 32 / NPER;
  constexpr int NL = MAXG * NPER;
  const int N = G * NPER, NS = N + 1 + (N & 1);
  float2* yt = compose_lds;
  float2* red = yt + SHF_TB * NS;
  float* sw = (float*)(red + N * SHF_TB);
  const int tile = blockIdx.x, k0 = tile * SHF_TB;
  const int nbin = K - k0 < SHF_TB ? K - k0 : SHF_TB;
  const size_t base = (size_t)k0 * N;
  for (int e = threadIdx.x; e < SHF_TB * N; e += 256) {
    const int kq = e / N, n = e - kq * N;
    yt[kq * NS + n] = e < nbin * N ? Y[base + e] : make_float2(0.f, 0.f);
  }
  for (int e = threadIdx.x; e < B * N; e += 256) sw[e] = w[e];
  __syncthreads();
  const int lane = threadIdx.x & 63, wv = threadIdx.x >> 6;
  const int k = k0 + lane;
  const bool valid = k < K;
  const int kk = valid ? k : K - 1;
  const float2 fc = filt ? cconj(filt[kk]) : make_float2(1.f, 0.f);
  const float2* yrow = yt + lane * NS;
  float2 acc[NL];
#pragma unroll
  for (int n = 0; n < NL; ++n) acc[n] = make_float2(0.f, 0.f);
  float* prow = partial + (size_t)tile * ((size_t)B * N + N);
  for (int b = wv; b < B; b += 4) {
    float2 gh[NPER];
#pragma unroll
    for (int l = 0; l < NPER; ++l) {
      float2 v = valid ? gH[((size_t)b * NPER + l) * K + kk] : make_float2(0.f, 0.f);
      if (filt) v = cmul(v, fc);
      gh[l] = v;
    }
    const float* swb = sw + b * N;
    float dot[NL];
#pragma unroll
    for (int g = 0; g < MAXG; ++g) {
#pragma unroll
      for (int l = 0; l < NPER; ++l) {
        const int n = g * NPER + l;
        dot[n] = 0.f;
        if (g < G) {
          const float s = swb[n];
          acc[n].x += s * gh[l].x;
          acc[n].y += s * gh[l].y;
          const float2 y = yrow[n];
          dot[n] = gh[l].x * y.x + gh[l].y * y.y;
        }
      }
    }
    static_assert(NL <= 32, "the halving exchange takes 32 values");
    const float mine = wave_sums_transposed32<NL>(dot);
    if (!(lane & 1) && (lane >> 1) < N) prow[(size_t)b * N + (lane >> 1)] = mine * c[lane >> 1];
  }
#pragma unroll 1
  for (int src = 3; src >= 1; --src) {
    if (wv == src) {
#pragma unroll
      for (int n = 0; n < NL; ++n) if (n < N) red[n * SHF_TB + lane] = acc[n];
    }
    __syncthreads();
    if (wv == src - 1) {
#pragma unroll
      for (int n = 0; n < NL; ++n) if (n < N) { const float2 o = red[n * SHF_TB + lane]; acc[n].x += o.x; acc[n].y += o.y; }
    }
    __syncthreads();
  }
  if (wv == 0) {
    float mine = 0.f;
#pragma unroll
    for (int n = 0; n < NL; ++n) {
      if (n < N) {
        const float2 a = acc[n];
        const float2 y = yrow[n];
        const float v = wave_sum(valid ? (a.x * y.x + a.y * y.y) : 0.f);
        if (lane == n) mine = v;
        yt[lane * NS + n] = cscale(a, c[n]);
      }
    }
    if (lane < N) prow[(size_t)B * N + lane] = mine;
  }
  __syncthreads();
  for (int e = threadIdx.x; e < nbin * N; e += 256) {
    const int kq = e / N, n = e - kq * N;
    gY[base + e] = yt[kq * NS + n];
  }
}

__global__ __launch_bounds__(256) void k_reduce_partials2(const float* __restrict__ partial, int nparts, int per1, int per2,
                                                          float* __restrict__ out1, float* __restrict__ out2) {
  __shared__ float s_red[16];
  const int e = blockIdx.x, per = per1 + per2;
  float s = 0.f;
  for (int p = threadIdx.x; p < nparts; p += 256) s += partial[(size_t)p * per + e];
  s = block_sum(s, s_red);
  if (threadIdx.x == 0) {
    if (e < per1) out1[e] = s;
    else out2[e - per1] = s;
  }
}

template <int NPER>
static int compose_sh_bwd_fused(const float2* Y, int K, int G, const float* c, const float* w, int B, const float2* filt,
                                const float2* gH, float2* gY, float* gc, float* gw, float* work, hipStream_t s) {
  const int N = G * NPER, NS = N + 1 + (N & 1), ntiles = (K + SHF_TB - 1) / SHF_TB;
  const size_t lds = ((size_t)SHF_TB * NS + (size_t)N * SHF_TB) * sizeof(float2) + (size_t)B * N * sizeof(float);
  int rc = ensure_dyn_lds(k_compose_sh_bwd_fused<NPER>, lds);
  if (rc) return rc;
  hipLaunchKernelGGL(k_compose_sh_bwd_fused<NPER>, dim3(ntiles), dim3(256), lds, s, Y, K, G, c, w, B, filt, gH, gY, work);
  GFDN_LAUNCH_CHECK();
  hipLaunchKernelGGL(k_reduce_partials2, dim3(B * N + N), dim3(256), 0, s, work, ntiles, B * N, N, gw, gc);
  GFDN_LAUNCH_CHECK();
  return 0;
}
static bool compose_sh_fused_ok(int K, int G, int nper, int B) {
  if (nper != 1 && nper != 4 && nper != 9 && nper != 16) return false;
  const int maxg = nper <= 4 ? 8 : 32 / nper;
  const int N = G * nper, NS = N + 1 + (N & 1);
  if (G > maxg || N > 64) return false;
  const size_t lds = ((size_t)SHF_TB * NS + (size_t)N * SHF_TB) * sizeof(float2) + (size_t)B * N * sizeof(float);
  return lds <= 64 * 1024 && (K + SHF_TB - 1) / SHF_TB <= GFDN_SH_MAX_TILES * (SH_TB / SHF_TB);
}

extern "C" size_t gfdn_compose_sh_bwd_work_bytes(int G, int nper, int B) {
  const size_t two_pass = ((size_t)(GFDN_SH_MAX_TILES * SH_TB / SH_KC) * B + GFDN_SH_MAX_TILES) * G * nper * sizeof(float);
  const size_t fused = (size_t)GFDN_SH_MAX_TILES * (SH_TB / SHF_TB) * ((size_t)B + 1) * G * nper * sizeof(float);
  return two_pass > fused ? two_pass : fused;
}

extern "C" int gfdn_compose_sh_bwd(const float* Y, int K, int G, int nper, const float* c,
                                   const float* w, int B, const float* filt, const float* gH,
                                   float* gY, float* gc, float* gw, void* work, void* stream) {
  if (!Y || !c || !w || !gH || !gY || !gc || !gw || !work) return GFDN_E_BADARG;
  if (K <= 0 || G <= 0 || nper <= 0 || B <= 0) return GFDN_E_BADARG;
  const int N = G * nper, NS = N + 1 + (N & 1);
  const int ntiles = (K + SH_TB - 1) / SH_TB, nchunks = (K + SH_KC - 1) / SH_KC;
  if (N > GFDN_MAX_SH_LINES || G > SH_TB || ntiles > GFDN_SH_MAX_TILES) return GFDN_E_UNSUPPORTED;
  const size_t lds = ((size_t)SH_TB * NS + (size_t)nper * SH_TB) * sizeof(float2) +
                     ((size_t)B * N + (size_t)(SH_TB / 64) * N + N) * sizeof(float);
  hipStream_t s = (hipStream_t)stream;
  if (compose_sh_fused_ok(K, G, nper, B)) {
    const float2 *Yc = (const float2*)Y, *fl = (const float2*)filt, *gh = (const float2*)gH;
    switch (nper) {
      case 1: return compose_sh_bwd_fused<1>(Yc, K, G, c, w, B, fl, gh, (float2*)gY, gc, gw, (float*)work, s);
// ... 255 lines not shown
```

### diffgfdn_amd/hip_ops.py

```python
import ctypes
from typing import Optional, Tuple

import torch

from . import _lib

_c64 = torch.complex64
_f32 = torch.float32


def _stream() -> int:
    return torch.cuda.current_stream().cuda_stream


def _need_gpu(*ts):
    for t in ts:
        if t is not None and not t.is_cuda:
            raise RuntimeError("diffgfdn_amd HIP ops need CUDA/HIP tensors (no CPU fallback)")


def _p(t: Optional[torch.Tensor]):
    return None if t is None else t.data_ptr()


# ... 431 lines not shown
            raise RuntimeError("subfdn_colorless_fwd: gains must be contiguous float32 of G*nper elements")
    K = turns.numel()
    lib = _lib.load()
    Y = torch.empty((K, G * nper), dtype=_c64, device=M.device)
    S = torch.empty((K, G), dtype=_c64, device=M.device)
    energy = torch.empty(G, dtype=_f32, device=M.device)
    work = _work(lib.gfdn_subfdn_colorless_work_bytes(G, nper), M.device)
    _lib.check(lib.gfdn_subfdn_colorless_fwd(_p(turns), _p(logr), K, G, nper, _p(M), _p(delays), _p(b), _p(c),
                                             int(bool(normalize)), _p(Y), _p(S), _p(energy), _p(work), _stream()),
               "gfdn_subfdn_colorless_fwd")
    return Y, S, energy


def spectral_stats_binmajor(S, energy, asym: bool, scale: float = 1.0, want_grad: bool = True):
    _need_gpu(S)
    S = _c(S)
    K, G = S.shape
    loss = torch.empty(G, dtype=_f32, device=S.device)
    gS = torch.empty_like(S) if want_grad else None
    lib = _lib.load()
    work = _work(lib.gfdn_subfdn_colorless_work_bytes(G, 4), S.device)
    _lib.check(lib.gfdn_spectral_stats_binmajor(_p(S), G, K, _p(energy), int(asym), float(scale), _p(loss), _p(gS),
                                                _p(work), _stream()), "gfdn_spectral_stats_binmajor")
    return loss, gS


def subfdn_colorless_bwd(turns, logr, M, delays, b, c, energy, Y, gS):
    _need_gpu(turns, M, Y, gS)
    M, delays, b, c = _f(M), _f(delays), _f(b), _f(c)
    G, nper, _ = M.shape
    K = turns.numel()
    if tuple(Y.shape) != (K, G * nper) or tuple(gS.shape) != (K, G):
        raise RuntimeError("subfdn_colorless_bwd: Y (K, G*nper) and gS (K, G) expected")
    lib = _lib.load()
    gM = torch.empty_like(M)
    gb = torch.empty(G * nper, dtype=_f32, device=M.device)
    gc = torch.empty_like(gb)
    work = _work(lib.gfdn_subfdn_colorless_work_bytes(G, nper), M.device)
    _lib.check(lib.gfdn_subfdn_colorless_bwd(_p(turns), _p(logr), K, G, nper, _p(M), _p(delays), _p(b), _p(c),
                                             _p(energy), _p(_c(Y)), _p(_c(gS)), _p(gM), _p(gb), _p(gc), _p(work),
                                             _stream()), "gfdn_subfdn_colorless_bwd")
    return gM, gb, gc


def normalize_io(energy, b, c, G: int, nper: int):
    _need_gpu(energy, b, c)
    for t in (b, c):
        if t.dtype != _f32 or not t.is_contiguous() or t.numel() != G * nper:
            raise RuntimeError("normalize_io: gains must be contiguous float32 of G*nper elements")
    _lib.check(_lib.load().gfdn_normalize_io(_p(energy), _p(b), _p(c), G, nper, _stream()),
               "gfdn_normalize_io")


def tf_coefs(A, b, c, inv_gamma=None, out=None) -> torch.Tensor:
    _need_gpu(A, b, c)
    A, b, c = _f(A), _f(b).reshape(-1), _f(c).reshape(-1)
    nblk, n, _ = A.shape
    if n > 4:
        raise RuntimeError("tf_coefs: blocks of at most 4 delay lines")
    if b.numel() != nblk * n or c.numel() != nblk * n:
        raise RuntimeError("tf_coefs: b, c must hold nblk * n gains")
    ig = None if inv_gamma is None else _f(inv_gamma).reshape(-1)
    if ig is not None and ig.numel() != nblk * n:
        raise RuntimeError("tf_coefs: inv_gamma must hold nblk * n gains")
    coef = torch.empty((nblk, 32), dtype=_f32, device=A.device) if out is None else out
    _lib.check(_lib.load().gfdn_tf_coefs_fwd(_p(A), _p(b), _p(c), _p(ig), nblk, n, _p(coef), _stream()),
               "gfdn_tf_coefs_fwd")
    return coef


def tf_coefs2(A0, ig0, A1, ig1, b, c):
    _need_gpu(A0, A1, b, c)
    A0, A1, b, c = _f(A0), _f(A1), _f(b).reshape(-1), _f(c).reshape(-1)
    nblk, n, _ = A0.shape
    if n > 4 or A1.shape != A0.shape or b.numel() != nblk * n or c.numel() != nblk * n:
        raise RuntimeError("tf_coefs2: two sets of nblk blocks of at most 4 lines, b, c of nblk * n gains")
    ig0 = None if ig0 is None else _f(ig0).reshape(-1)
    ig1 = None if ig1 is None else _f(ig1).reshape(-1)
    c0 = torch.empty((nblk, 32), dtype=_f32, device=A0.device)
    c1 = torch.empty((nblk, 32), dtype=_f32, device=A0.device)
    _lib.check(_lib.load().gfdn_tf_coefs_fwd2(_p(A0), _p(ig0), _p(c0), _p(A1), _p(ig1), _p(c1), _p(b), _p(c), nblk, n,
                                              _stream()), "gfdn_tf_coefs_fwd2")
    return c0, c1


def tf_parts(K: int, nblk: int) -> int:
    n = _lib.load().gfdn_tf_parts(int(K), int(nblk))
    if n <= 0:
        raise RuntimeError("tf_parts: unsupported number of blocks")
    return n


def tf_gpart(nblk: int, device) -> torch.Tensor:
    return torch.empty(_lib.load().gfdn_tf_gpart_bytes(nblk) // 4, dtype=_f32, device=device)


def tf_eval(turns, logr, coef, delays, nper: int, scale=None) -> torch.Tensor:
    _need_gpu(turns, coef, delays)
    coef, delays = _f(coef), _f(delays)
    nblk, K = coef.shape[0], turns.numel()
    if delays.numel() != nblk * nper:
        raise RuntimeError("tf_eval: delays must hold nblk * nper entries")
    scale = None if scale is None else _f(scale)
    T = torch.empty((K, nblk), dtype=_c64, device=coef.device)
    _lib.check(_lib.load().gfdn_tf_eval(_p(turns), _p(logr), K, nblk, nper, _p(coef), _p(delays), _p(scale), _p(T),
                                        _stream()), "gfdn_tf_eval")
    return T


def tf_energy(turns, logr, coef, delays, nper: int, b=None, c=None, want_energy=True, want_scale=True, work=None,
              phase: int = 3, energy=None, scale=None, dturn: float = 0.0, gains=None, G: int = 0):
    _need_gpu(turns, coef, delays)
    coef, delays = _f(coef), _f(delays)
    nblk, K = coef.shape[0], turns.numel()
    for t in (b, c):
        if t is not None and (t.dtype != _f32 or not t.is_contiguous() or t.numel() != nblk * nper):
            raise RuntimeError("tf_energy: gains must be contiguous float32 of nblk*nper elements")
    lib = _lib.load()
    if phase & 2:
        energy = torch.empty(nblk, dtype=_f32, device=coef.device) if (want_energy and energy is None) else energy
        scale = torch.empty(nblk, dtype=_f32, device=coef.device) if (want_scale and scale is None) else scale
    work = _work(lib.gfdn_tf_work_bytes(nblk), coef.device) if work is None else work
    if gains is not None:
        if not (phase & 2) or G <= 0 or nblk % G or gains.dtype != _f32 or not gains.is_contiguous() or gains.shape[1] != G \
                or gains.shape[0] % (nblk // G):
            raise RuntimeError("tf_energy: gains (bands * Bper, G) float32 contiguous with nblk = bands * G, with the finish")
        gs = torch.empty_like(gains)
        _lib.check(lib.gfdn_tf_energy_gains(_p(turns), _p(logr), K, nblk, nper, _p(coef), _p(delays), _p(b), _p(c), _p(energy),
                                            _p(scale), _p(work), int(phase), float(dturn), _p(gains), _p(gs),
                                            gains.shape[0] // (nblk // G), G, _stream()), "gfdn_tf_energy_gains")
        return energy, scale, gs
    _lib.check(lib.gfdn_tf_energy(_p(turns), _p(logr), K, nblk, nper, _p(coef), _p(delays), _p(b), _p(c), _p(energy),
                                  _p(scale), _p(work), int(phase), float(dturn), _stream()), "gfdn_tf_energy")
    return work if phase == 1 else (energy, scale)


def tf_colorless(turns, logr, coef, delays, nper: int, scale, asym: bool, gscale: float, work=None,
                 dturn: float = 0.0):
    _need_gpu(turns, coef, delays)
    coef, delays = _f(coef), _f(delays)
    nblk, K = coef.shape[0], turns.numel()
    scale = None if scale is None else _f(scale)
    work = tf_gpart(nblk, coef.device) if work is None else work
    grec = torch.empty((nblk, 32), dtype=_f32, device=coef.device)
    loss = torch.empty(nblk, dtype=_f32, device=coef.device)
    _lib.check(_lib.load().gfdn_tf_colorless(_p(turns), _p(logr), K, nblk, nper, _p(coef), _p(delays), _p(scale),
                                             int(asym), float(gscale), _p(grec), _p(loss), _p(work), float(dturn),
                                             _stream()),
               "gfdn_tf_colorless")
    return grec, loss


def tf_compose_fwd(turns, logr, coef, delays, nper: int, rgain, scale=None, direct=None, filt=None,
                   direct_rows=None, nbands: int = 1, out=None, save_T: bool = False, want_H: bool = True):
    _need_gpu(turns, coef, rgain)
    coef, delays, rgain = _f(coef), _f(delays), _f(rgain)
    K = turns.numel()
    Btot, G = rgain.shape
    if coef.shape[0] != nbands * G or Btot % nbands or delays.numel() != nbands * G * nper:
        raise RuntimeError("tf_compose_fwd: shapes do not match nbands x G blocks")
    ldd = 0
    if direct is not None:
        direct = direct.detach()
        if not (direct.dtype == _c64 and direct.dim() == 2 and direct.stride(1) == 1 and direct.stride(0) >= K
                and direct.shape[1] >= K):
            direct = _c(direct)
        ldd = direct.stride(0)
    filt = None if filt is None else _c(filt)
    if filt is not None and filt.numel() != nbands * K:
        raise RuntimeError("tf_compose_fwd: filt must hold K bins per band")
    direct_rows = None if direct is None else _rows(direct_rows, Btot, direct.shape[0])
    if direct is not None and direct_rows is None and direct.shape[0] != Btot:
        raise RuntimeError("tf_compose_fwd: direct must have one row per item (or pass direct_rows)")
    scale = None if scale is None else _f(scale)
    if not want_H and not save_T:
        raise RuntimeError("tf_compose_fwd: nothing to compute")
    H = None if not want_H else (torch.empty((Btot, K), dtype=_c64, device=coef.device) if out is None else out)
    Ts = torch.empty((nbands * G, K), dtype=_c64, device=coef.device) if save_T else None
    Tq = torch.empty((nbands, K, 4), dtype=_c64, device=coef.device) if not want_H else None
    _lib.check(_lib.load().gfdn_tf_compose_fwd(_p(turns), _p(logr), K, nbands, G, nper, _p(coef), _p(delays),
                                               _p(scale), _p(rgain), Btot // nbands, _p(direct), ldd,
                                               _p(direct_rows), _p(filt), K, _p(H), K, _p(Ts), _p(Tq), _stream()),
               "gfdn_tf_compose_fwd")
    if not want_H:
        return Tq, Ts
    return (H, Ts) if save_T else H


def tf_gain_grad(Tsave, gH, G: int, filt=None, nbands: int = 1, grgain=None, work=None, partial: bool = False):
    _need_gpu(Tsave, gH)
    Tsave, gH = _c(Tsave), _c(gH)
    Btot, K = gH.shape
    if Btot % nbands or tuple(Tsave.shape) != (nbands * G, K):
        raise RuntimeError("tf_gain_grad: shapes do not match nbands x G blocks")
    filt = None if filt is None else _c(filt)
    lib = _lib.load()
    B = Btot // nbands
    if partial:
        parts = torch.empty((Btot * G, lib.gfdn_tf_gain_chunks(K)), dtype=_f32, device=gH.device)
        _lib.check(lib.gfdn_tf_gain_grad(K, nbands, G, B, _p(Tsave), _p(filt), K, _p(gH), K, None, _p(parts), _stream()),
                   "gfdn_tf_gain_grad")
        return parts
    grgain = torch.empty((Btot, G), dtype=_f32, device=gH.device) if grgain is None else grgain
    if work is None:
        work = _work(lib.gfdn_tf_gain_grad_work_bytes(K, nbands, G, B), gH.device)
    _lib.check(lib.gfdn_tf_gain_grad(K, nbands, G, B, _p(Tsave), _p(filt), K, _p(gH), K, _p(grgain), _p(work),
                                     _stream()), "gfdn_tf_gain_grad")
    return grgain


def tf_compose_bwd(turns, logr, coef, delays, nper: int, rgain, gH, Tsave, filt=None, nbands: int = 1, work=None,
                   partial: bool = False, tscale=None, gain_fold: bool = False):
    _need_gpu(turns, coef, rgain, gH, Tsave)
    if tscale is not None and (tscale.dtype != _f32 or not tscale.is_contiguous() or tscale.numel() != coef.shape[0]):
        raise RuntimeError("tf_compose_bwd: tscale must be a contiguous float32 vector with one factor per block")
    coef, delays, rgain, gH, Tsave = _f(coef), _f(delays), _f(rgain), _c(gH), _c(Tsave)
    K = turns.numel()
    Btot, G = rgain.shape
    if coef.shape[0] != nbands * G or Btot % nbands or tuple(gH.shape) != (Btot, K) \
            or tuple(Tsave.shape) != (nbands * G, K):
        raise RuntimeError("tf_compose_bwd: shapes do not match nbands x G blocks")
    filt = None if filt is None else _c(filt)
    lib = _lib.load()
    if partial:
        grec = None
        work = torch.empty((nbands * G, 32, lib.gfdn_tf_compose_parts(K)), dtype=_f32, device=coef.device)
    else:
        grec = torch.empty((nbands * G, 32), dtype=_f32, device=coef.device)
        if work is None:
            work = _work(lib.gfdn_tf_compose_bwd_work_bytes(K, nbands, G), coef.device)
    _lib.check(lib.gfdn_tf_compose_bwd(_p(turns), _p(logr), K, nbands, G, nper, _p(coef), _p(delays), _p(Tsave),
                                       _p(tscale), _p(rgain), Btot // nbands, _p(filt), K, _p(gH), K, _p(grec), _p(work),
                                       int(bool(gain_fold)), _stream()), "gfdn_tf_compose_bwd")
    return work if partial else grec


def tf_param_grads(A0, ig0, grec0, b, c, M, A1=None, ig1=None, grec1=None, gQ=None, Q=None, gb=None, gc=None, gM=None):
    _need_gpu(A0, grec0, b, c, M)
    A0, b, c, grec0, M = _f(A0), _f(b).reshape(-1), _f(c).reshape(-1), _f(grec0), _f(M)
    nblk, n, _ = A0.shape
    nparts0 = 1 if grec0.dim() == 2 else grec0.shape[2]
    if tuple(grec0.shape[:2]) != (nblk, 32) or (grec1 is not None and tuple(grec1.shape) != (nblk, 32)) \
            or tuple(M.shape) != (nblk, n, n):
        raise RuntimeError("tf_param_grads: records must be (nblk, 32[, parts]), M (nblk, n, n)")
    dev = A0.device
    ig0 = None if ig0 is None else _f(ig0).reshape(-1)
    if A1 is not None:
        A1, grec1 = _f(A1), _f(grec1)
        ig1 = None if ig1 is None else _f(ig1).reshape(-1)
    gb = torch.empty(nblk * n, dtype=_f32, device=dev) if gb is None else gb
    gc = torch.empty(nblk * n, dtype=_f32, device=dev) if gc is None else gc
    gM = torch.empty_like(M) if gM is None else gM
    _lib.check(_lib.load().gfdn_tf_param_grads(_p(A0), _p(ig0), _p(grec0), nparts0, _p(A1), _p(ig1), _p(grec1), _p(b),
                                               _p(c), nblk, n, _p(M), _p(None if gQ is None else _f(gQ)),
                                               _p(None if Q is None else _f(Q)), _p(gb), _p(gc), _p(gM), _stream()),
               "gfdn_tf_param_grads")
    return gM, gb, gc


def tf_tail(QQ, ig, grec0, grec1, b, c, M, gQ, Q, gb, gc, gM, opt, offM: int, offb: int, offc: int, Q_next, QQ_next,
            coef_next, coef_sub_next):
    _need_gpu(QQ, grec0, b, c, M)
    nblk, n, _ = QQ.shape
    nparts0 = 1 if grec0.dim() == 2 else grec0.shape[2]
    ig = None if ig is None else _f(ig).reshape(-1)
    for t in (QQ, grec0, grec1, b, c, M, gQ, Q, gb, gc, gM, Q_next, QQ_next, coef_next, coef_sub_next):
        if t is not None and (t.dtype != _f32 or not t.is_contiguous()):
            raise RuntimeError("tf_tail: contiguous float32 tensors expected")
    if tuple(grec0.shape[:2]) != (nblk, 32) or tuple(grec1.shape) != (nblk, 32) or M.numel() != nblk * n * n \
            or b.numel() != nblk * n or c.numel() != nblk * n:
        raise RuntimeError("tf_tail: records must be (nblk, 32[, parts]), M (nblk, n, n), b / c (nblk n)")
    fp = opt.flat_param
    for off, t in ((offM, M), (offb, b), (offc, c)):
        if fp.data_ptr() + 4 * off != t.data_ptr():
            raise RuntimeError("tf_tail: the leaves must be the flat buffer's views at the stated offsets")
    b1, b2 = opt.defaults['betas']
    _lib.check(_lib.load().gfdn_tf_tail(_p(QQ), _p(ig), _p(grec0), nparts0, _p(M), _p(grec1), _p(b), _p(c), nblk, n, _p(M),
                                        _p(gQ), _p(Q), _p(gb), _p(gc), _p(gM), _p(fp), _p(opt.exp_avg), _p(opt.exp_avg_sq),
                                        _p(opt.seg), _p(opt.lr_seg), _p(opt.step_count), _p(opt._block_counter), int(offM),
                                        int(offb), int(offc), float(b1), float(b2), float(opt.defaults['eps']),
                                        _p(Q_next), _p(QQ_next), _p(coef_next), _p(coef_sub_next), _stream()),
               "gfdn_tf_tail")


def tf_ortho_coefs(M, ig, b, c, sub: bool = True, out=None):
    _need_gpu(M, b, c)
    M, b, c = _f(M), _f(b).reshape(-1), _f(c).reshape(-1)
    nblk, n, _ = M.shape
    ig = None if ig is None else _f(ig).reshape(-1)
    if out is not None:
        Q, QQ, coef, coef_sub = out
    else:
        Q, QQ = torch.empty_like(M), torch.empty_like(M)
        coef = torch.empty((nblk, 32), dtype=_f32, device=M.device)
        coef_sub = torch.empty((nblk, 32), dtype=_f32, device=M.device) if sub else None
    _lib.check(_lib.load().gfdn_tf_ortho_coefs(_p(M), _p(ig), _p(b), _p(c), nblk, n, _p(Q), _p(QQ), _p(coef),
                                               _p(coef_sub), _stream()), "gfdn_tf_ortho_coefs")
    return Q, QQ, coef, coef_sub


def tf8_coefs(A0, ig0, b, c, A1=None, ig1=None):
    _need_gpu(A0, b, c)
    A0, b, c = _f(A0), _f(b).reshape(-1), _f(c).reshape(-1)
    nblk, n, _ = A0.shape
    if b.numel() != nblk * n or c.numel() != nblk * n:
        raise RuntimeError("tf8_coefs: b, c must hold nblk * n gains")
    ig0 = None if ig0 is None else _f(ig0).reshape(-1)
    c0 = torch.empty((nblk, 9, 256), dtype=_f32, device=A0.device)
    c1 = None
    if A1 is not None:
        A1 = _f(A1)
        ig1 = None if ig1 is None else _f(ig1).reshape(-1)
        c1 = torch.empty((nblk, 9, 256), dtype=_f32, device=A0.device)
    _lib.check(_lib.load().gfdn_tf8_coefs(_p(A0), _p(ig0), _p(c0), _p(A1), _p(ig1), _p(c1), _p(b), _p(c), nblk, n,
                                          _stream()), "gfdn_tf8_coefs")
    return c0, c1


def tf8_parts(K: int) -> int:
    return _lib.load().gfdn_tf8_parts(int(K))


def tf8_energy(turns, coef, delays, nper: int, b, c, want_energy: bool = False, dturn: float = 0.0):
    _need_gpu(turns, coef, delays, b, c)
    coef, delays = _f(coef), _f(delays)
    nblk, K = coef.shape[0], turns.numel()
    for t in (b, c):
        if t.dtype != _f32 or not t.is_contiguous() or t.numel() != nblk * nper:
            raise RuntimeError("tf8_energy: gains must be contiguous float32 of nblk * nper elements")
    lib = _lib.load()
    energy = torch.empty(nblk, dtype=_f32, device=coef.device) if want_energy else None
    scale = torch.empty(nblk, dtype=_f32, device=coef.device)
    work = torch.empty(nblk * lib.gfdn_tf8_parts(K), dtype=_f32, device=coef.device)
    _lib.check(lib.gfdn_tf8_energy(_p(turns), K, nblk, nper, _p(coef), _p(delays), _p(b), _p(c), _p(energy), _p(scale),
                                   _p(work), float(dturn), _stream()), "gfdn_tf8_energy")
    return energy, scale


def tf8_tsave(turns, coef, delays, nper: int, c, scale, nbands: int, G: int, quad: bool = True, filt=None,
              want_H: bool = False, hslot=None):
    _need_gpu(turns, coef, delays, c)
    coef, delays, c = _f(coef), _f(delays), _f(c).reshape(-1)
    K = turns.numel()
    if coef.shape[0] != nbands * G:
        raise RuntimeError("tf8_tsave: records do not match nbands x G blocks")
    scale = None if scale is None else _f(scale)
    filt = None if filt is None else _c(filt)
    if filt is not None and filt.numel() != nbands * K:
        raise RuntimeError("tf8_tsave: filt must hold K bins per band")
    Ts = torch.empty((nbands * G, K), dtype=_c64, device=coef.device)
    Tq = torch.empty((nbands, K, 4), dtype=_c64, device=coef.device) if quad else None
    Hg = torch.empty((nbands * G, K), dtype=_c64, device=coef.device) if want_H else None
    Dinv = torch.empty((nbands * G, K), dtype=_c64, device=coef.device) if want_H else None
    _lib.check(_lib.load().gfdn_tf8_tsave(_p(turns), K, nbands, G, nper, _p(coef), _p(delays), _p(c), _p(scale), _p(Ts),
                                          _p(Tq), _p(filt if want_H else None), K, _p(Hg), _p(Dinv),
                                          _p(hslot if want_H else None), _stream()), "gfdn_tf8_tsave")
    return (Ts, Tq, Hg, Dinv) if want_H else (Ts, Tq)


def tf8_colorless(turns, coef, delays, nper: int, c, scale, asym: bool, gscale: float, dturn: float = 0.0):
    _need_gpu(turns, coef, delays, c)
    coef, delays, c = _f(coef), _f(delays), _f(c).reshape(-1)
    nblk, K = coef.shape[0], turns.numel()
    lib = _lib.load()
    parts = lib.gfdn_tf8_parts(K)
    part = torch.empty((nblk, 512, parts), dtype=_f32, device=coef.device)
    lossp = torch.empty((nblk, parts), dtype=_f32, device=coef.device)
    loss = torch.empty(nblk, dtype=_f32, device=coef.device)
    _lib.check(lib.gfdn_tf8_colorless(_p(turns), K, nblk, nper, _p(coef), _p(delays), _p(c), _p(None if scale is None else _f(scale)),
                                      int(asym), float(gscale), _p(part), _p(lossp), _p(loss), float(dturn), _stream()),
               "gfdn_tf8_colorless")
    return part, loss


def tf8_compose_bwd(turns, coef, delays, nper: int, c, scale, rgain, gH, filt=None, nbands: int = 1, saved=None):
    _need_gpu(turns, coef, delays, c, rgain, gH)
    coef, delays, c, rgain, gH = _f(coef), _f(delays), _f(c).reshape(-1), _f(rgain), _c(gH)
    K = turns.numel()
    Btot, G = rgain.shape
    if coef.shape[0] != nbands * G or Btot % nbands or gH.shape[0] != Btot or gH.shape[1] < K:
        raise RuntimeError("tf8_compose_bwd: shapes do not match nbands x G blocks")
    filt = None if filt is None else _c(filt)
    if filt is not None and filt.numel() != nbands * K:
        raise RuntimeError("tf8_compose_bwd: filt must hold K bins per band")
    lib = _lib.load()
    part = torch.empty((nbands * G, 512, lib.gfdn_tf8_parts(K)), dtype=_f32, device=coef.device)
# ... 1580 lines not shown
```

### include/diffgfdn_hip.h

```cpp
#ifndef DIFFGFDN_HIP_H
#define DIFFGFDN_HIP_H

#include <stddef.h>
#include <stdint.h>

#ifdef __cplusplus
extern "C" {
#endif

#define GFDN_ABI_VERSION 8
#define GFDN_E_BADARG (-1)
#define GFDN_E_UNSUPPORTED (-2)
#define GFDN_MAX_BLOCK 32
#define GFDN_MAX_GROUPS 8
#define GFDN_PARTIAL_BLOCKS 256

int gfdn_abi_version(void);

int gfdn_zprep(const double* z_c128, int K, double* turns, double* logr, void* stream);

int gfdn_ortho_fwd(const float* M, int G, int n, float* Q, float* QQ, void* stream);
int gfdn_ortho_bwd(const float* M, int G, int n, const float* gQ, const float* gQQ, const float* Q,
                   float* gM, void* stream);
int gfdn_ortho_bwd_add(const float* M, int G, int n, const float* gQ, const float* gQQ, const float* Q,
// ... 11 lines not shown
size_t gfdn_solve_bwd_work_bytes(int nblk, int nper);
int gfdn_solve_bwd(const double* turns, const double* logr, int K, int nblk, int nper,
                   const float* A, const float* delays, const float* inv_gamma,
                   const float* b, int transpose, const float* gY_c64, const float* Y_c64,
                   float* gA, float* gb, float* ginv_gamma, void* work, void* stream);

int gfdn_solve_precise_fwd(const double* turns, const double* logr, int K, int nblk, int nper,
                           const float* A, const float* delays, const double* inv_gamma_f64, const float* b,
                           int transpose, float* Y_c64, void* stream);
int gfdn_solve_precise_bwd(const double* turns, const double* logr, int K, int nblk, int nper,
                           const float* A, const float* delays, const double* inv_gamma_f64, const float* b,
                           int transpose, const float* gY_c64, const float* Y_c64, float* gA, float* gb,
                           float* ginv_gamma, void* work, void* stream);

int gfdn_solve_absorb_fwd(const double* turns, const double* logr, int K, int nblk, int nper,
                          const float* A, const float* delays, const float* ones,
                          const float* inv_gamma_bins_c64, const float* b, int transpose, float* Y_c64,
                          void* stream);
int gfdn_solve_absorb_bwd(const double* turns, const double* logr, int K, int nblk, int nper,
                          const float* A, const float* delays, const float* ones,
                          const float* inv_gamma_bins_c64, const float* b, int transpose,
                          const float* gY_c64, const float* Y_c64, float* gA, float* gb,
                          float* ginv_scratch, void* work, void* stream);

int gfdn_solve_phi_fwd(const double* turns, const double* logr, int K, int G, int nper, const float* BM,
                       const float* Phi_c64, const float* delays, const float* inv_gamma, const float* b,
                       float* Y_c64, void* stream);
size_t gfdn_solve_phi_bwd_work_bytes(int G, int nper);
int gfdn_solve_phi_bwd(const double* turns, const double* logr, int K, int G, int nper, const float* BM,
                       const float* Phi_c64, const float* delays, const float* inv_gamma, const float* b,
                       const float* gY_c64, const float* Y_c64, float* gBM, float* gb, float* ginv_gamma,
                       float* gPhi_c64, void* work, void* stream);
int gfdn_solve_phi_absorb_fwd(const double* turns, const double* logr, int K, int G, int nper, const float* BM,
                              const float* Phi_c64, const float* delays, const float* inv_gamma,
                              const float* inv_gamma_bins_c64, const float* b, float* Y_c64, void* stream);
int gfdn_solve_phi_absorb_bwd(const double* turns, const double* logr, int K, int G, int nper, const float* BM,
                              const float* Phi_c64, const float* delays, const float* inv_gamma,
                              const float* inv_gamma_bins_c64, const float* b, const float* gY_c64,
                              const float* Y_c64, float* gBM, float* gb, float* ginv_gamma, float* gPhi_c64,
                              void* work, void* stream);

int gfdn_svf_coefficients(const float* raw, const double* cutoff, double compress_pole_factor, int R, int S,
                          const float* gcoef, float* out, void* stream);
int gfdn_sos_response(const float* coef, int R, int S, const double* z_c128, int K, float* out_c64, void* stream);
int gfdn_sos_compose_fwd(const float* coef, int B, int G, int S, const double* z_c128, int K, const float* T_c64,
                         const float* direct_c64, int ldd, float* H_c64, void* stream);
int gfdn_sos_compose_bwd_chunks(int B, int K, int* t_chunks, int* c_chunks);
int gfdn_sos_compose_bwd(const float* coef, int B, int G, int S, const double* z_c128, int K, const float* T_c64,
                         const float* gH_c64, float* gT_partial_c64, float* gcoef_partial, void* stream);

int gfdn_compose_fwd(const float* Y_c64, int K, int G, int nper, const float* c,
                     const float* rgain, int B, const float* direct_c64, int ldd,
                     const long long* direct_rows, const float* filt_c64, float* H_c64, int ldh,
                     float* S_out_c64, void* stream);

size_t gfdn_compose_bwd_work_bytes(int K, int G, int nper, int B);
int gfdn_compose_bwd(const float* Y_c64, int K, int G, int nper, const float* c,
                     const float* rgain, int B, const float* filt_c64, const float* gH_c64,
                     int ldh, float* gY_c64, float* gc, float* grgain, void* work, void* stream);

int gfdn_compose_banded_fwd(const float* Y_c64, int K, int nbands, int G, int nper, const float* c,
                            const float* rgain, int B, const float* direct_c64, int ldd,
                            const long long* direct_rows, const float* filt_c64, int ldf,
                            float* H_c64, int ldh, float* S_out_c64, void* stream);
size_t gfdn_compose_banded_bwd_work_bytes(int K, int nbands, int G, int nper, int B);
int gfdn_compose_banded_bwd(const float* Y_c64, int K, int nbands, int G, int nper, const float* c,
                            const float* rgain, int B, const float* filt_c64, int ldf,
                            const float* gH_c64, int ldh, float* gY_c64, float* gc, float* grgain,
                            void* work, void* stream);

int gfdn_compose_sh_fwd(const float* Y_c64, int K, int G, int nper, const float* c,
                        const float* w, int B, const float* filt_c64, float* H_c64,
                        void* stream);
size_t gfdn_compose_sh_bwd_work_bytes(int G, int nper, int B);
int gfdn_compose_sh_bwd(const float* Y_c64, int K, int G, int nper, const float* c,
                        const float* w, int B, const float* filt_c64, const float* gH_c64,
                        float* gY_c64, float* gc, float* gw, void* work, void* stream);

int gfdn_sh_to_directional(const float* A, int J, int C, int K, int B, const float* in_c64,
                           float* out_c64, int adjoint, void* stream);

size_t gfdn_spectral_stats_work_bytes(int G, int K);
int gfdn_spectral_stats(const float* S_c64, int G, int K, int asym, float scale,
                        float* energy, float* loss, float* gS_c64, void* work, void* stream);

int gfdn_colorless_terms(const float* loss_g, int G, const float* Q, int n, float w_spec,
                         float w_sparse, float inv_world, float* out3, float* gQ, void* stream);
int gfdn_colorless_terms_banded(const float* loss_g, int nbands, int G, const float* Q, int n,
                                float w_spec, float w_sparse, float inv_world, float* out3, float* gQ,
                                void* stream);
int gfdn_weighted_sums(const float* a, int a_cols, const float* a_div, const long long* a_rows,
                       float wa, const float* b, float wb, int n, float* out3, void* stream);

int gfdn_weighted_sums_banded(const float* a, int a_cols, const float* a_div, const long long* a_rows,
                              float wa, const float* b, float wb, int n, int nbands, float* out3,
                              void* stream);

int gfdn_normalize_io(const float* energy, float* b, float* c, int G, int nper, void* stream);

size_t gfdn_subfdn_normalize_work_bytes(int G);
int gfdn_subfdn_normalize(const double* turns, const double* logr, int K, int G, int nper,
                          const float* M, const float* delays, float* b, float* c, float* energy,
                          void* work, void* stream);

size_t gfdn_subfdn_colorless_work_bytes(int G, int nper);
int gfdn_subfdn_colorless_fwd(const double* turns, const double* logr, int K, int G, int nper,
                              const float* M, const float* delays, float* b, float* c, int normalize,
                              float* Y_c64, float* S_c64, float* energy, void* work, void* stream);
int gfdn_spectral_stats_binmajor(const float* S_c64, int G, int K, const float* energy, int asym,
                                 float scale, float* loss, float* gS_c64, void* work, void* stream);
int gfdn_subfdn_colorless_bwd(const double* turns, const double* logr, int K, int G, int nper,
                              const float* M, const float* delays, const float* b, const float* c,
                              const float* energy, const float* Y_c64, const float* gS_c64, float* gM,
                              float* gb, float* gc, void* work, void* stream);

int gfdn_tf_coefs_fwd(const float* A, const float* b, const float* c, const float* inv_gamma, int nblk,
                      int nper, float* coef, void* stream);
int gfdn_tf_coefs_fwd2(const float* A0, const float* inv_gamma0, float* coef0, const float* A1,
                       const float* inv_gamma1, float* coef1, const float* b, const float* c, int nblk, int nper,
                       void* stream);
int gfdn_tf_ortho_coefs(const float* M, const float* inv_gamma, const float* b, const float* c, int nblk, int nper,
                        float* Q, float* QQ, float* coef, float* coef_sub, void* stream);
int gfdn_tf_coefs_bwd(const float* A0, const float* inv_gamma0, const float* grec0, const float* A1,
                      const float* inv_gamma1, const float* grec1, const float* b, const float* c, int nblk,
                      int nper, float* gA0, float* gA1, float* gb, float* gc, void* stream);
int gfdn_tf_param_grads(const float* A0, const float* inv_gamma0, const float* grec0, int nparts0, const float* A1,
                        const float* inv_gamma1, const float* grec1, const float* b, const float* c, int nblk,
                        int nper, const float* M, const float* gQ, const float* Q, float* gb, float* gc, float* gM,
                        void* stream);
int gfdn_tf_tail(const float* A0, const float* inv_gamma0, const float* grec0, int nparts0, const float* A1,
                 const float* grec1, const float* b, const float* c, int nblk, int nper, const float* M, const float* gQ,
                 const float* Q, float* gb, float* gc, float* gM, float* flat_p, float* flat_m, float* flat_v,
                 const unsigned char* seg, const float* lr_seg, float* step_count, unsigned int* block_counter, int offM,
                 int offb, int offc, float beta1, float beta2, float eps, float* Q_next, float* QQ_next, float* coef_next,
                 float* coef_sub_next, void* stream);
int gfdn_tf_rows_sum(const float* part, int cols, int rows, float* out, void* stream);
int gfdn_tf_parts(int K, int nblk);
size_t gfdn_tf_work_bytes(int nblk);
size_t gfdn_tf_gpart_bytes(int nblk);
int gfdn_tf_eval(const double* turns, const double* logr, int K, int nblk, int nper, const float* coef,
                 const float* delays, const float* scale, float* T_c64, void* stream);
int gfdn_tf_energy(const double* turns, const double* logr, int K, int nblk, int nper, const float* coef,
                   const float* delays, float* b, float* c, float* energy, float* scale, void* work,
                   int phase, double dturn, void* stream);
int gfdn_tf_energy_gains(const double* turns, const double* logr, int K, int nblk, int nper, const float* coef,
                         const float* delays, float* b, float* c, float* energy, float* scale, void* work, int phase,
                         double dturn, const float* gains, float* gains_scaled, int Bper, int G, void* stream);
int gfdn_tf_colorless(const double* turns, const double* logr, int K, int nblk, int nper, const float* coef,
                      const float* delays, const float* scale, int asym, float gscale, float* grec,
                      float* loss, void* work, double dturn, void* stream);
int gfdn_tf_compose_fwd(const double* turns, const double* logr, int K, int nbands, int G, int nper,
                        const float* coef, const float* delays, const float* scale, const float* rgain, int B,
                        const float* direct_c64, int ldd, const long long* direct_rows, const float* filt_c64,
                        int ldf, float* H_c64, int ldh, float* Tsave_c64, float* Tquad_c64, void* stream);
int gfdn_tf_compose_parts(int K);
size_t gfdn_tf_compose_bwd_work_bytes(int K, int nbands, int G);
int gfdn_tf_compose_bwd(const double* turns, const double* logr, int K, int nbands, int G, int nper,
                        const float* coef, const float* delays, const float* Tsave_c64, const float* tscale,
                        const float* rgain, int B, const float* filt_c64, int ldf, const float* gH_c64, int ldh,
                        float* grec, void* work, int gain_fold, void* stream);
size_t gfdn_tf_gain_grad_work_bytes(int K, int nbands, int G, int B);
int gfdn_tf_gain_grad(int K, int nbands, int G, int B, const float* Tsave_c64, const float* filt_c64, int ldf,
                      const float* gH_c64, int ldh, float* grgain, void* work, void* stream);
int gfdn_tf_gain_chunks(int K);

int gfdn_tf8_coefs(const float* A0, const float* inv_gamma0, float* coef0, const float* A1, const float* inv_gamma1,
                   float* coef1, const float* b, const float* c, int nblk, int nper, void* stream);
int gfdn_tf8_parts(int K);
size_t gfdn_tf8_part_bytes(int nblk, int K);
int gfdn_tf8_energy(const double* turns, int K, int nblk, int nper, const float* coef, const float* delays, float* b,
                    float* c, float* energy, float* scale, void* work, double dturn, void* stream);
int gfdn_tf8_tsave(const double* turns, int K, int nbands, int G, int nper, const float* coef, const float* delays,
                   const float* c, const float* scale, float* Tsave_c64, float* Tquad_c64, const float* filt_c64, int ldf,
                   float* Hout_c64, float* Dinv_c64, const int* hslot, void* stream);
int gfdn_tf8_colorless(const double* turns, int K, int nblk, int nper, const float* coef, const float* delays,
                       const float* c, const float* scale, int asym, float gscale, float* part, float* lossp,
                       float* loss, double dturn, void* stream);
int gfdn_tf8_compose_bwd(const double* turns, int K, int nbands, int G, int nper, const float* coef, const float* delays,
                         const float* c, const float* scale, const float* rgain, int B, const float* filt_c64, int ldf,
                         const float* gH_c64, int ldh, const float* Tsave_c64, const float* Dinv_c64, float* part,
                         void* stream);
size_t gfdn_tf8_param_grads_work_bytes(int nblk);
int gfdn_tf8_param_grads(const float* A0, const float* inv_gamma0, const float* part0, int nparts0, const float* A1,
                         const float* inv_gamma1, const float* part1, int nparts1, const float* b, const float* c,
                         int nblk, int nper, const float* M, const float* gQ, const float* Q, float* gb, float* gc,
                         float* gM, void* work, void* stream);
int gfdn_tf8_tail(const float* A0, const float* inv_gamma0, const float* part0, int nparts0, const float* A1, const float* part1,
                  int nparts1, const float* b, const float* c, int nblk, int nper, const float* M, const float* gQ,
                  const float* Q, float* gb, float* gc, float* gM, void* work, float* flat_p, float* flat_m, float* flat_v,
                  const unsigned char* seg, const float* lr_seg, float* step_count, unsigned int* block_counter, int offM,
                  int offb, int offc, float beta1, float beta2, float eps, float* Q_next, float* QQ_next, float* c_next,
                  void* stream);
int gfdn_tf9_coefs(const float* A, const float* inv_gamma, const float* b, int nblk, int nper, float* coef, void* stream);
size_t gfdn_tf9_rec_grads_work_bytes(int nblk);
int gfdn_tf9_rec_grads(const float* A, const float* inv_gamma, const float* grec, const float* b, const float* c, int nblk,
                       int nper, float* gA, float* gb, float* gc, void* work, void* stream);
int gfdn_tfp_ratio_fwd(const float* Xq_c64, const float* Xp_c64, int ldx, int K, int nblk, float* T_c64, float* Dinv_c64,
                       void* stream);
int gfdn_tfp_ratio_bwd(int nfft, int nblk, int nper, int nsub, const float* delays, const float* gT_c64, int ldg, const float* T_c64,
                       const float* Dinv_c64, int T, float* UV_c64, int ldx, float* x, int ldt, void* work, float* part,
                       void* stream);
int gfdn_tfp_parts(void);
int gfdn_tfp_forward(int nfft, int nblk, int nper, int nsub, const float* coef, const float* delays, const float* c, int T,
                     float* seq, float* X_c64, int ldx, void* work, void* stream);
int gfdn_tfp_energy(const float* Xq_c64, const float* Xp_c64, int ldx, int K, int nblk, int nper, float* b, float* c,
                    float* energy, float* scale, void* work, const float* gains, float* gains_scaled, int Bper, int G,
                    void* stream);
int gfdn_tfp_colorless(const float* Xq_c64, const float* Xp_c64, int ldx, int nfft, int nblk, int nper, const float* delays,
                       const float* scale, int asym, float gscale, int T, float* UV_c64, float* x, int ldt, void* work,
                       float* part, float* lossp, float* loss, void* stream);
int gfdn_tfp_compose_bwd(int nfft, int nbands, int G, int nper, const float* delays, int Ku, const int* slot_of_bin,
                         const float* gH_c64, int ldh, const float* filt_c64, int ldf, const float* Tnat_c64,
                         const float* Dnat_c64, const float* tscale, int gain_fold, int T, float* UV_c64, int ldx, float* x,
                         int ldt, void* work, float* part, void* stream);

int gfdn_exp_contract_mfma(const float* P_c64, int K, const float* C, const float* bvec, int use_bf16,
                           float* H_c64, void* stream);

size_t gfdn_bluestein_table_bytes(int n);
int gfdn_bluestein_table_init(int n, void* table);
size_t gfdn_bluestein_work_bytes(int n, int batch);
int gfdn_irfft_odd_fwd(const void* table, int n, const float* X_c64, int ldx, int batch,
                       float* x, int ldo, void* work, void* stream);
int gfdn_irfft_odd_bwd(const void* table, int n, const float* gx, const float* gx2, int ldo,
                       int batch, float* gX_c64, int ldx, void* work, void* stream);

int gfdn_irfft_odd_slot_order(int n, int* bins_host, int* conj_host);
int gfdn_irfft_odd_slots_fwd(const void* table, int n, const float* Xs_c64, int ldx, int batch,
                             float* x, int ldo, void* work, void* stream);
int gfdn_irfft_odd_slots_bwd(const void* table, int n, const float* gx, const float* gx2, int ldo,
                             int batch, float* gXs_c64, int ldx, void* work, void* stream);

int gfdn_irfft_odd_pairs_fwd(const void* table, int n, const float* Xs_c64, int ldx, int batch,
                             float* x2, int ldo, void* work, void* stream);
int gfdn_irfft_odd_pairs_compose_fwd(const void* table, int n, const float* direct_c64, int ldd,
                                     const long long* direct_rows, const float* T_c64, int ldt, const float* rgain,
                                     const float* filt_c64, int ldf, int nbands, int G, int batch, float* h0,
                                     float* x2, int ldo, void* work, int stages, void* stream);
int gfdn_irfft_odd_pairs_bwd(const void* table, int n, const float* gx2, const float* gx2b, int ldo,
                             int batch, float* gXs_c64, int ldx, void* work, void* stream);
int gfdn_irfft_odd_pairs_gains_parts(int n);
int gfdn_irfft_odd_pairs_gains_bwd(const void* table, int n, const float* gx2, const float* gx2b, int ldo, int batch,
                                   float* gXs_c64, int ldx, const float* T_c64, int ldt, const float* filt_c64, int ldf,
                                   int nbands, int G, float* gpart, void* work, int stages, void* stream);
int gfdn_stft_power_pairs(const float* x2, int ld, int T, int items, int win, float* P, float* zero_buf2,
                          void* stream);
int gfdn_stft_power_pairs_bwd(const float* x2, int ld, int T, int items, int win, const float* gP,
                              const float* base2, float* gx2, void* stream);
int gfdn_stft_power_pairs_bwd_phase(const float* x2, int ld, int T, int items, int win, const float* gP,
                                    const float* base2, float* gx2, int phase, void* stream);
int gfdn_edc_loss_pairs(const float* x2, int ld, int items, int start, int len, const float* T_db,
                        const long long* target_rows, const float* maskw, float inv_count, float gscale,
                        float* loss_item, float* gx2, void* work, void* stream);

int gfdn_lin_gain_chunks(int n);
int gfdn_lin_combine_fwd(const float* xd, int ld_xd, const long long* rows, const float* tau, int ld_tau, int tau_pairs,
                         const float* rgain, int nbands, int B, int G, int n, float* x, int ld_x, int out_pairs,
                         void* stream);
int gfdn_lin_gamma(const float* gx, const float* gxb, int ld_g, int in_pairs, const float* rgain, int nbands, int B, int G,
                   int n, float* gamma, int ld_o, int out_pairs, const int* slot_of_time, const float* base2, int ld_b,
                   void* stream);
int gfdn_irfft_odd_time_slots(int n, int* times);
int gfdn_irfft_odd_pairs_bwd_tslots(const void* table, int n, const float* gx2s, int ldo, int batch, float* gXs_c64,
                                    int ldx, void* work, void* stream);
int gfdn_irfft_odd_pairs_bwd_tslots3(const void* table, int n, const float* gx2s_a, const float* gx2s_b,
                                     const float* gx2s_c, int ldo, int batch, float* gXs_c64, int ldx, void* work,
                                     void* stream);
int gfdn_irfft_odd_pairs_fwd_scaled(const void* table, int n, const float* Xs_c64, int ldx, int batch, const float* oscale,
                                    float* x2, int ldo, void* work, int stages, void* stream);
int gfdn_lin_gain_dots(const float* gx, const float* gxb, int ld_g, int in_pairs, const float* tau, int ld_tau,
                       int tau_pairs, int nbands, int B, int G, int n, float* part, int ld_part, void* stream);

int gfdn_lin_gamma_dots_tiles(int n);
int gfdn_lin_gamma_dots(const float* gx2, int ld_g, const float* rgain, int nbands, int B, int G, int n, const float* tau2,
                        int ld_tau, const float* base2, int ld_b, const int* slot_of_time, float* gamma, int ld_o,
                        float* part, int ld_part, int win_start, int win_len, const int* band_win_len, const float* base2b,
                        void* stream);

int gfdn_stft_pairs_spectrum(const float* x2, int ld, int T, int items, int win, float* S_c64, int tiled, void* stream);
int gfdn_stft_pairs_spectrum_bwd(const float* G_c64, int T, int items, int win, const float* base2, float* gx2, int ld,
                                 int tiled, int nsplit, float* gx2b, void* stream);
int gfdn_edr_lin_parts(int nfreq);
int gfdn_edr_lin_band_parts(int nfreq);
int gfdn_edr_lin_loss(const float* Sd_c64, const long long* rows, const float* Stau_c64, const float* rgain, int nbands,
                      int B, int G, const float* T_db, const float* sum_abs, int nframes, int nfreq, float gscale,
                      int want_grad, float* gP, float* part, float* dots, int ld_dots, int col0, int tiled, void* stream);
int gfdn_edr_lin_gsum(const float* Sd_c64, const long long* rows, const float* Stau_c64, const float* rgain, int nbands,
                      int B, int G, const float* gP, int nframes, int nfreq, float* Gsum_c64, void* stream);
int gfdn_edr_lin_loss_gsum(const float* Sd_c64, const long long* rows, const float* Stau_c64, const float* rgain, int nbands,
                           int B, int G, const float* T_db, const float* sum_abs, int nframes, int nfreq, float gscale,
                           float* part, int ld_part, float* dots, int ld_dots, int col0, float* Gsum_c64, int nsplit,
                           int tiled, void* stream);
int gfdn_edc_loss_pairs_lin(const float* xd, int ld_xd, const long long* xrows, const float* tau2, int ld_tau,
                            const float* rgain, int nbands, int B, int G, int ld, int start, int max_len,
                            const int* item_len, const float* T_db, int ld_T, const long long* target_rows,
                            const float* maskw, int ld_mask, float inv_count, float gscale, float* loss_item, float* gx2,
                            int fill_outside, float* xwin2, void* work, void* stream);

int gfdn_edc_lin_one_max_len(void);
int gfdn_edc_lin_one(const float* xd, int ld_xd, const long long* xrows, const float* tau2, int ld_tau, const float* rgain,
                     int nbands, int B, int G, int start, int max_len, const int* item_len, const float* T_db, int ld_T,
                     const long long* target_rows, const float* maskw, int ld_mask, float inv_count, float gscale,
                     float* loss_item, float* gx, int ld_gx, float* dots, int ld_dots, int col, void* stream);
int gfdn_lin_gamma_win(const float* gx, int ld_g, const float* rgain, int nbands, int B, int G, int n, int win_start,
                       int win_len, const int* band_win_len, const float* base2a, const float* base2b, int ld_b,
                       const int* slot_of_time, float* gamma2, int ld_o, void* stream);

int gfdn_lin_merge_slots(const float* a2, const float* b2, const float* c2, int rows, int n, int ld, const int* slot_of_time,
                         float* out2, int ld_o, void* stream);

size_t gfdn_f64_fft_work_bytes(int rows, int M);
int gfdn_irfft_odd_f64_length(int n);
int gfdn_rfft_pow2_f64(const double* x, int ldx, int len, int rows, int nfft, double* X_c128, int kout, void* work,
// ... 142 lines not shown
```

Baseline: 21.80 million.

## Use phasor rotation runs and identity-gain path in transfer-function compose kernels

Forward and backward transfer-function compose kernels gain a 'runs' variant for uniform unit-circle grids. It computes the delay phasors z^-m once per thread and gets later bins by multiplying with precomputed rotation factors held in shared memory, which avoids a transcendental evaluation per bin. The backward kernel also gets an identity-gain specialization that reads one gH row instead of reducing over B gains. Its final per-wave reductions now use a shared transposed permlane/DPP sum instead of 32 separate wave sums. Chaining rotations in f32 across a run can add rounding error, and the forward runs kernel uses 64-thread blocks, which changes occupancy.

```diff
diff --git a/diffgfdn_amd/_lib.py b/diffgfdn_amd/_lib.py
--- a/diffgfdn_amd/_lib.py
+++ b/diffgfdn_amd/_lib.py
@@ -79,11 +79,11 @@
                                      _P]),
     "gfdn_tf_colorless": (c_int, [_P, _P, c_int, c_int, c_int, _P, _P, _P, c_int, c_float, _P, _P, _P, c_double, _P]),
     "gfdn_tf_compose_fwd": (c_int, [_P, _P, c_int, c_int, c_int, c_int, _P, _P, _P, _P, c_int, _P, c_int, _P, _P, c_int, _P, c_int, _P, _P,
-                                    _P]),
+                                    c_double, _P]),
     "gfdn_tf_compose_parts": (c_int, [c_int]),
     "gfdn_tf_compose_bwd_work_bytes": (c_size_t, [c_int, c_int, c_int]),
     "gfdn_tf_compose_bwd": (c_int, [_P, _P, c_int, c_int, c_int, c_int, _P, _P, _P, _P, _P, c_int, _P, c_int, _P, c_int, _P, _P,
-                                    c_int, _P]),
+                                    c_int, c_double, _P]),
     "gfdn_tf_tail": (c_int, [_P, _P, _P, c_int, _P, _P, _P, _P, c_int, c_int, _P, _P, _P, _P, _P, _P, _P, _P, _P, _P, _P, _P,
                              _P, c_int, c_int, c_int, c_float, c_float, c_float, _P, _P, _P, _P, _P]),
     "gfdn_irfft_odd_pairs_bwd_tslots3": (c_int, [_P, c_int, _P, _P, _P, c_int, c_int, _P, c_int, _P, _P]),
diff --git a/diffgfdn_amd/bankstep.py b/diffgfdn_amd/bankstep.py
--- a/diffgfdn_amd/bankstep.py
+++ b/diffgfdn_amd/bankstep.py
@@ -249,7 +249,7 @@
         if p.late:
             st.Hg, st.Ts = ops.tf_compose_fwd(gridU.turns, gridU.logr, st.coef, st.delays, p.n,
                                               self._eye_rows(p.nb, p.G, st.rows.device), None, None, st.filt, None, p.nb,
-                                              save_T=True, want_H=True)
+                                              save_T=True, want_H=True, dturn=gridU.dturn)
         if p.late8:
             st.Ts, _, st.Hg, st.Dinv8 = ops.tf8_tsave(gridK.turns[:p.Ku], st.coef, st.delays, p.n, st.c_head, None, p.nb, p.G,
                                                       quad=False, filt=st.filt, want_H=True, hslot=p.tfp[1])
@@ -320,7 +320,7 @@
             st.ev_ts.record()
         elif not p.late:
             st.Hg, st.Ts = ops.tf_compose_fwd(gridU.turns, gridU.logr, st.coef, st.delays, p.n, st.eye, st.scale, None,
-                                              st.filt, None, p.nb, save_T=True, want_H=True)
+                                              st.filt, None, p.nb, save_T=True, want_H=True, dturn=gridU.dturn)
         if p.gfold:
             st.tau = ops.irfft_odd_fwd(st.Hg, K, slots=True, pairs=True)
         elif p.late or p.late8:
@@ -350,7 +350,7 @@
                 st.H = Hs.reshape(p.Btot, -1).contiguous()
         else:
             st.H, st.Ts = ops.tf_compose_fwd(gridU.turns, gridU.logr, st.coef, st.delays, p.n, st.rgain, st.scale, st.direct,
-                                             st.filt, st.rows, p.nb, save_T=True, want_H=not p.fold)
+                                             st.filt, st.rows, p.nb, save_T=True, want_H=not p.fold, dturn=gridU.dturn)
         if p.fold:
             st.Tq, st.H = st.H, None
 
@@ -523,7 +523,7 @@
         else:
             st.grec = ops.tf_compose_bwd(gridU.turns, gridU.logr, st.coef, st.delays, p.n, st.rg_rec, st.gH_rec, st.Ts, st.filt,
                                          p.nb, partial=True, tscale=st.scale if p.late else None,
-                                         gain_fold=p.gfold and p.late)
+                                         gain_fold=p.gfold and p.late, dturn=gridU.dturn, identity=p.lin)
 
     def _side_backward(self, p: "_Plan", st: "_Step"):
         tr, ev, pipe = self.tr, st.ev, st.pipe
diff --git a/diffgfdn_amd/csrc/blocktf.hip b/diffgfdn_amd/csrc/blocktf.hip
--- a/diffgfdn_amd/csrc/blocktf.hip
+++ b/diffgfdn_amd/csrc/blocktf.hip
@@ -852,21 +852,12 @@
 };
 
 #define TFC_BCH 8
-__global__ __launch_bounds__(256) void k_tf_compose_fwd(TfCompose a, const float2* __restrict__ direct, int ldd,
-                                                        const long long* __restrict__ drows,
-                                                        float2* __restrict__ H, int ldh, float2* __restrict__ Tsave,
-                                                        float2* __restrict__ Tquad) {
-  __shared__ TfBlock tab[TF_MAXG];
-  const int band = blockIdx.y, G = a.G, B = a.B;
-  tf_stage(a.coef, a.delays, band * G, G, a.nper, tab);
-  __syncthreads();
-  const int k = blockIdx.x * 256 + threadIdx.x;
-  if (k >= a.K) return;
-  const float* rgain = a.rgain + (size_t)band * B * G;
-  if (drows) drows += (size_t)band * B;
-  else if (direct) direct += (size_t)band * B * ldd;
-  if (H) H += (size_t)band * B * ldh;
-  else direct = nullptr;
+template <class PH>
+__device__ __forceinline__ void tfc_bin(const TfCompose& a, const TfBlock* tab, int band, int k, const float* rgain,
+                                        const float2* __restrict__ direct, int ldd, const long long* __restrict__ drows,
+                                        float2* __restrict__ H, int ldh, float2* __restrict__ Tsave,
+                                        float2* __restrict__ Tquad, PH&& phasors) {
+  const int G = a.G, B = a.B;
   float2 d[TFC_BCH];
 #pragma unroll
   for (int bb = 0; bb < TFC_BCH; ++bb)
@@ -877,7 +868,8 @@
     T[g] = make_float2(0.f, 0.f);
     if (g < G) {
       float2 e[16], num, den;
-      tf_phasors(a.turns, a.logr, k, tab[g].m, e);
+      phasors(g, e);
+      tf_subsets(e);
       tf_numden(tab[g].P, tab[g].Q, e, num, den);
       T[g] = cmul(num, cinv(den));
       if (a.scale) T[g] = cscale(T[g], a.scale[band * G + g]);
@@ -920,6 +912,67 @@
   }
 }
 
+__global__ __launch_bounds__(256) void k_tf_compose_fwd(TfCompose a, const float2* __restrict__ direct, int ldd,
+                                                        const long long* __restrict__ drows,
+                                                        float2* __restrict__ H, int ldh, float2* __restrict__ Tsave,
+                                                        float2* __restrict__ Tquad) {
+  __shared__ TfBlock tab[TF_MAXG];
+  const int band = blockIdx.y, G = a.G, B = a.B;
+  tf_stage(a.coef, a.delays, band * G, G, a.nper, tab);
+  __syncthreads();
+  const int k = blockIdx.x * 256 + threadIdx.x;
+  if (k >= a.K) return;
+  const float* rgain = a.rgain + (size_t)band * B * G;
+  if (drows) drows += (size_t)band * B;
+  else if (direct) direct += (size_t)band * B * ldd;
+  if (H) H += (size_t)band * B * ldh;
+  else direct = nullptr;
+  tfc_bin(a, tab, band, k, rgain, direct, ldd, drows, H, ldh, Tsave, Tquad, [&](int g, float2 (&e)[16]) {
+    e[1] = tf_zpow(a.turns, a.logr, k, tab[g].m[0]);
+    e[2] = tf_zpow(a.turns, a.logr, k, tab[g].m[1]);
+    e[4] = tf_zpow(a.turns, a.logr, k, tab[g].m[2]);
+    e[8] = tf_zpow(a.turns, a.logr, k, tab[g].m[3]);
+  });
+}
+
+#define TFC_RUN 4
+__global__ __launch_bounds__(64) void k_tf_compose_fwd_runs(TfCompose a, double dturn, const float2* __restrict__ direct,
+                                                            int ldd, const long long* __restrict__ drows,
+                                                            float2* __restrict__ H, int ldh, float2* __restrict__ Tsave,
+                                                            float2* __restrict__ Tquad) {
+  __shared__ TfBlock tab[TF_MAXG];
+  __shared__ float2 rot[TFC_RUN][TF_MAXG * 4];
+  const int band = blockIdx.y, G = a.G, B = a.B;
+  tf_stage(a.coef, a.delays, band * G, G, a.nper, tab);
+  __syncthreads();
+  for (int t = threadIdx.x; t < (TFC_RUN - 1) * TF_MAXG * 4; t += 64) {
+    const int j = 1 + t / (TF_MAXG * 4), q = t % (TF_MAXG * 4);
+    rot[j][q] = (q >> 2) < G ? tf_rot(dturn * (double)(64 * j), tab[q >> 2].m[q & 3]) : make_float2(1.f, 0.f);
+  }
+  __syncthreads();
+  const int k0 = blockIdx.x * (64 * TFC_RUN) + threadIdx.x;
+  if (k0 >= a.K) return;
+  const float* rgain = a.rgain + (size_t)band * B * G;
+  if (drows) drows += (size_t)band * B;
+  else if (direct) direct += (size_t)band * B * ldd;
+  if (H) H += (size_t)band * B * ldh;
+  else direct = nullptr;
+  float2 seed[TF_MAXG][4];
+#pragma unroll 1
+  for (int j = 0; j < TFC_RUN; ++j) {
+    const int k = k0 + 64 * j;
+    if (k >= a.K) break;
+    tfc_bin(a, tab, band, k, rgain, direct, ldd, drows, H, ldh, Tsave, Tquad, [&](int g, float2 (&e)[16]) {
+      if (j == 0) {
+#pragma unroll
+        for (int i = 0; i < 4; ++i) seed[g][i] = tf_zpow(a.turns, nullptr, k0, tab[g].m[i]);
+      }
+#pragma unroll
+      for (int i = 0; i < 4; ++i) e[1 << i] = j == 0 ? seed[g][i] : cmul(seed[g][i], rot[j][4 * g + i]);
+    });
+  }
+}
+
 static int tf_compose_ok(const double* turns, int K, int nbands, int G, int nper, int B, const float* coef,
                          const float* delays, const float* rgain) {
   if (!turns || !coef || !delays || !rgain || K <= 0 || nbands <= 0 || G <= 0 || nper <= 0 || B <= 0)
@@ -932,14 +985,19 @@
                                    const float* coef, const float* delays, const float* scale,
                                    const float* rgain, int B, const float* direct, int ldd,
                                    const long long* direct_rows, const float* filt, int ldf, float* H, int ldh,
-                                   float* Tsave, float* Tquad, void* stream) {
+                                   float* Tsave, float* Tquad, double dturn, void* stream) {
   int rc = tf_compose_ok(turns, K, nbands, G, nper, B, coef, delays, rgain);
   if (rc) return rc;
   if ((!H && !Tsave && !Tquad) || (H && ldh < K) || (direct && ldd < K) || (filt && nbands > 1 && ldf < K)) return GFDN_E_BADARG;
   TfCompose a{turns, logr, K, G, nper, B, coef, delays, scale, rgain, (const float2*)filt, ldf};
-  hipLaunchKernelGGL(k_tf_compose_fwd, dim3((K + 255) / 256, nbands), dim3(256), 0, (hipStream_t)stream, a,
-                     (const float2*)direct, ldd, direct ? direct_rows : nullptr, (float2*)H, ldh, (float2*)Tsave,
-                     (float2*)Tquad);
+  if (dturn != 0.0 && !logr)
+    hipLaunchKernelGGL(k_tf_compose_fwd_runs, dim3((K + 64 * TFC_RUN - 1) / (64 * TFC_RUN), nbands), dim3(64), 0,
+                       (hipStream_t)stream, a, dturn, (const float2*)direct, ldd, direct ? direct_rows : nullptr, (float2*)H,
+                       ldh, (float2*)Tsave, (float2*)Tquad);
+  else
+    hipLaunchKernelGGL(k_tf_compose_fwd, dim3((K + 255) / 256, nbands), dim3(256), 0, (hipStream_t)stream, a,
+                       (const float2*)direct, ldd, direct ? direct_rows : nullptr, (float2*)H, ldh, (float2*)Tsave,
+                       (float2*)Tquad);
   GFDN_LAUNCH_CHECK();
   return 0;
 }
@@ -994,16 +1052,26 @@
 }
 
 #define TFR_BCH 8
-__global__ __launch_bounds__(256) void k_tf_compose_bwd_rec(TfCompose a, const float2* __restrict__ Tsave,
+#define TFR_RUN 4
+template <bool RUNS, bool EYE>
+__global__ __launch_bounds__(256) void k_tf_compose_bwd_rec(TfCompose a, double dturn, const float2* __restrict__ Tsave,
                                                             const float2* __restrict__ gH, int ldh,
                                                             float* __restrict__ gpart) {
   __shared__ TfBlock tab[TF_MAXG];
+  __shared__ float2 rot[TFR_RUN][TF_MAXG * 4];
   const int band = blockIdx.y, G = a.G, B = a.B, nparts = gridDim.x;
   tf_stage(a.coef, a.delays, band * G, G, a.nper, tab);
   __syncthreads();
+  if (RUNS) {
+    for (int t = threadIdx.x; t < (TFR_RUN - 1) * TF_MAXG * 4; t += 256) {
+      const int j = 1 + t / (TF_MAXG * 4), q = t % (TF_MAXG * 4);
+      rot[j][q] = (q >> 2) < G ? tf_rot(dturn * (64.0 * nparts * j), tab[q >> 2].m[q & 3]) : make_float2(1.f, 0.f);
+    }
+    __syncthreads();
+  }
   const int lane = threadIdx.x & 63, w = __builtin_amdgcn_readfirstlane(threadIdx.x >> 6);
   if (w >= G) return;
-  const float* rgain = a.rgain + (size_t)band * B * G + w;
+  const float* rgain = EYE ? nullptr : a.rgain + (size_t)band * B * G + w;
   gH += (size_t)band * B * ldh;
   const float2* Tp = Tsave + (size_t)(band * G + w) * a.K;
   float Q[16], m[4];
@@ -1017,26 +1085,43 @@
   const float tsc = a.scale ? a.scale[band * G + w] : 1.0f;
   const float itsc = 1.0f / tsc;
   const int ntiles = (a.K + TFB_T - 1) / TFB_T;
+  float2 seed[4];
+  int j = 0;
   for (int tile = blockIdx.x; tile < ntiles; tile += nparts) {
     const int k = tile * TFB_T + lane;
     const bool live = k < a.K;
     const int kk = live ? k : a.K - 1;
     float2 acc = make_float2(0.f, 0.f);
-    for (int b0 = 0; b0 < B; b0 += TFR_BCH) {
-      float2 gh[TFR_BCH];
-#pragma unroll
-      for (int i = 0; i < TFR_BCH; ++i)
-        gh[i] = (live && b0 + i < B) ? gH[(size_t)(b0 + i) * ldh + kk] : make_float2(0.f, 0.f);
-#pragma unroll
-      for (int i = 0; i < TFR_BCH; ++i) {
-        const float rg = b0 + i < B ? rgain[(b0 + i) * G] : 0.f;
-        acc.x += rg * gh[i].x;
-        acc.y += rg * gh[i].y;
+    if (EYE) {
+      if (live) acc = gH[(size_t)w * ldh + kk];
+    } else {
+      for (int b0 = 0; b0 < B; b0 += TFR_BCH) {
+        float2 gh[TFR_BCH];
+#pragma unroll
+        for (int i = 0; i < TFR_BCH; ++i)
+          gh[i] = (live && b0 + i < B) ? gH[(size_t)(b0 + i) * ldh + kk] : make_float2(0.f, 0.f);
+#pragma unroll
+        for (int i = 0; i < TFR_BCH; ++i) {
+          const float rg = b0 + i < B ? rgain[(b0 + i) * G] : 0.f;
+          acc.x += rg * gh[i].x;
+          acc.y += rg * gh[i].y;
+        }
       }
     }
     if (a.filt) acc = cmulc(acc, a.filt[(size_t)band * a.ldf + kk]);
     float2 e[16];
-    tf_phasors(a.turns, a.logr, kk, m, e);
+    if (RUNS) {
+      if (j == 0) {
+#pragma unroll
+        for (int i = 0; i < 4; ++i) seed[i] = tf_zpow(a.turns, nullptr, kk, m[i]);
+      }
+#pragma unroll
+      for (int i = 0; i < 4; ++i) e[1 << i] = j == 0 ? seed[i] : cmul(seed[i], rot[j][4 * w + i]);
+      tf_subsets(e);
+      j = j + 1 < TFR_RUN ? j + 1 : 0;
+    } else {
+      tf_phasors(a.turns, a.logr, kk, m, e);
+    }
     float2 den = make_float2(Q[0], 0.f);
 #pragma unroll
     for (int S = 1; S < 16; ++S) {
@@ -1044,6 +1129,7 @@
       den.y += Q[S] * e[S].y;
     }
     float2 u = cmulc(acc, cinv(den));
+    if (RUNS && !live) u = make_float2(0.f, 0.f);
     float2 v;
     if (a.fold) {
       v = cmulc(u, Tp[kk]);
@@ -1060,14 +1146,14 @@
     }
   }
   float* out = gpart + (size_t)(band * G + w) * TF_REC * nparts + blockIdx.x;
+  float acc32[32];
 #pragma unroll
   for (int S = 0; S < 16; ++S) {
-    const float p = wave_sum_full(aP[S]), q = wave_sum_full(aQ[S]);
-    if (lane == 0) {
-      out[(size_t)S * nparts] = p;
-      out[(size_t)(16 + S) * nparts] = q;
-    }
-  }
+    acc32[S] = aP[S];
+    acc32[16 + S] = aQ[S];
+  }
+  const float mine = wave_sums_transposed32<32>(acc32);
+  if (!(lane & 1)) out[(size_t)(lane >> 1) * nparts] = mine;
 }
 
 static int tf_compose_parts_host(int K) {
@@ -1114,15 +1200,24 @@
 extern "C" int gfdn_tf_compose_bwd(const double* turns, const double* logr, int K, int nbands, int G, int nper,
                                    const float* coef, const float* delays, const float* Tsave, const float* tscale,
                                    const float* rgain, int B, const float* filt, int ldf, const float* gH,
-                                   int ldh, float* grec, void* work, int gain_fold, void* stream) {
-  int rc = tf_compose_ok(turns, K, nbands, G, nper, B, coef, delays, rgain);
+                                   int ldh, float* grec, void* work, int gain_fold, double dturn, void* stream) {
+  int rc = tf_compose_ok(turns, K, nbands, G, nper, B, coef, delays, rgain ? rgain : coef);
   if (rc) return rc;
-  if (!Tsave || !gH || !work || ldh < K || (filt && nbands > 1 && ldf < K) || (gain_fold && !tscale)) return GFDN_E_BADARG;
+  if (!Tsave || !gH || !work || ldh < K || (filt && nbands > 1 && ldf < K) || (gain_fold && !tscale) || (!rgain && B != G))
+    return GFDN_E_BADARG;
   TfCompose a{turns, logr, K, G, nper, B, coef, delays, tscale, rgain, (const float2*)filt, ldf, gain_fold ? 1 : 0};
   const int nparts = tf_compose_parts_host(K);
   hipStream_t s = (hipStream_t)stream;
-  hipLaunchKernelGGL(k_tf_compose_bwd_rec, dim3(nparts, nbands), dim3(256), 0, s, a, (const float2*)Tsave,
-                     (const float2*)gH, ldh, (float*)work);
+  const dim3 grid(nparts, nbands);
+  const bool runs = dturn != 0.0 && !logr;
+#define TFR_LAUNCH(RUNS, EYE)                                                                                       \
+  hipLaunchKernelGGL((k_tf_compose_bwd_rec<RUNS, EYE>), grid, dim3(256), 0, s, a, dturn, (const float2*)Tsave,      \
+                     (const float2*)gH, ldh, (float*)work)
+  if (runs && !rgain) TFR_LAUNCH(true, true);
+  else if (runs) TFR_LAUNCH(true, false);
+  else if (!rgain) TFR_LAUNCH(false, true);
+  else TFR_LAUNCH(false, false);
+#undef TFR_LAUNCH
   GFDN_LAUNCH_CHECK();
   if (!grec) return 0;
   const int n0 = nbands * G * TF_REC;
diff --git a/diffgfdn_amd/csrc/common.h b/diffgfdn_amd/csrc/common.h
--- a/diffgfdn_amd/csrc/common.h
+++ b/diffgfdn_amd/csrc/common.h
@@ -88,6 +88,45 @@
 #pragma unroll
   for (int off = 32; off >= 1; off >>= 1) v += __shfl_xor(v, off, 64);
   return v;
+}
+
+template <int NV>
+__device__ __forceinline__ float wave_sums_transposed32(const float (&v)[NV]) {
+  const int lane = threadIdx.x & 63;
+  float a[16];
+#pragma unroll
+  for (int i = 0; i < 16; ++i) {
+    const unsigned lo_v = __float_as_uint(i < NV ? v[i < NV ? i : 0] : 0.f);
+    const unsigned hi_v = __float_as_uint(i + 16 < NV ? v[i + 16 < NV ? i + 16 : 0] : 0.f);
+    const auto r = __builtin_amdgcn_permlane32_swap(lo_v, hi_v, false, false);
+    a[i] = __uint_as_float(r[0]) + __uint_as_float(r[1]);
+  }
+#pragma unroll
+  for (int i = 0; i < 8; ++i) {
+    const auto r = __builtin_amdgcn_permlane16_swap(__float_as_uint(a[i]), __float_as_uint(a[i + 8]), false, false);
+    a[i] = __uint_as_float(r[0]) + __uint_as_float(r[1]);
+  }
+  {
+    const bool hi = lane & 8;
+#pragma unroll
+    for (int i = 0; i < 4; ++i) {
+      const float s0 = dpp_pair_sum<0x128>(a[i]), s1 = dpp_pair_sum<0x128>(a[i + 4]);
+      a[i] = hi ? s1 : s0;
+    }
+  }
+  {
+    const bool hi = lane & 4;
+#pragma unroll
+    for (int i = 0; i < 2; ++i) {
+      const float s0 = dpp_pair_sum<0x141>(a[i]), s1 = dpp_pair_sum<0x141>(a[i + 2]);
+      a[i] = hi ? s1 : s0;
+    }
+  }
+  {
+    const float s0 = dpp_pair_sum<0x4e>(a[0]), s1 = dpp_pair_sum<0x4e>(a[1]);
+    a[0] = (lane & 2) ? s1 : s0;
+  }
+  return dpp_pair_sum<0xb1>(a[0]);
 }
 
 template <int CTRL>
diff --git a/diffgfdn_amd/csrc/solve.hip b/diffgfdn_amd/csrc/solve.hip
--- a/diffgfdn_amd/csrc/solve.hip
+++ b/diffgfdn_amd/csrc/solve.hip
@@ -2381,45 +2381,6 @@
   }
 }
 
-template <int NV>
-__device__ __forceinline__ float wave_sums_transposed32(const float (&v)[NV]) {
-  const int lane = threadIdx.x & 63;
-  float a[16];
-#pragma unroll
-  for (int i = 0; i < 16; ++i) {
-    const unsigned lo_v = __float_as_uint(i < NV ? v[i < NV ? i : 0] : 0.f);
-    const unsigned hi_v = __float_as_uint(i + 16 < NV ? v[i + 16 < NV ? i + 16 : 0] : 0.f);
-    const auto r = __builtin_amdgcn_permlane32_swap(lo_v, hi_v, false, false);
-    a[i] = __uint_as_float(r[0]) + __uint_as_float(r[1]);
-  }
-#pragma unroll
-  for (int i = 0; i < 8; ++i) {
-    const auto r = __builtin_amdgcn_permlane16_swap(__float_as_uint(a[i]), __float_as_uint(a[i + 8]), false, false);
-    a[i] = __uint_as_float(r[0]) + __uint_as_float(r[1]);
-  }
-  {
-    const bool hi = lane & 8;
-#pragma unroll
-    for (int i = 0; i < 4; ++i) {
-      const float s0 = dpp_pair_sum<0x128>(a[i]), s1 = dpp_pair_sum<0x128>(a[i + 4]);
-      a[i] = hi ? s1 : s0;
-    }
-  }
-  {
-    const bool hi = lane & 4;
-#pragma unroll
-    for (int i = 0; i < 2; ++i) {
-      const float s0 = dpp_pair_sum<0x141>(a[i]), s1 = dpp_pair_sum<0x141>(a[i + 2]);
-      a[i] = hi ? s1 : s0;
-    }
-  }
-  {
-    const float s0 = dpp_pair_sum<0x4e>(a[0]), s1 = dpp_pair_sum<0x4e>(a[1]);
-    a[0] = (lane & 2) ? s1 : s0;
-  }
-  return dpp_pair_sum<0xb1>(a[0]);
-}
-
 #define SHF_TB 64
 template <int NPER>
 __global__ __launch_bounds__(256, NPER <= 9 ? 4 : 2) void k_compose_sh_bwd_fused(const float2* __restrict__ Y, int K, int G,
diff --git a/diffgfdn_amd/hip_ops.py b/diffgfdn_amd/hip_ops.py
--- a/diffgfdn_amd/hip_ops.py
+++ b/diffgfdn_amd/hip_ops.py
@@ -607,7 +607,8 @@
 
 
 def tf_compose_fwd(turns, logr, coef, delays, nper: int, rgain, scale=None, direct=None, filt=None,
-                   direct_rows=None, nbands: int = 1, out=None, save_T: bool = False, want_H: bool = True):
+                   direct_rows=None, nbands: int = 1, out=None, save_T: bool = False, want_H: bool = True,
+                   dturn: float = 0.0):
     _need_gpu(turns, coef, rgain)
     coef, delays, rgain = _f(coef), _f(delays), _f(rgain)
     K = turns.numel()
@@ -635,7 +636,8 @@
     Tq = torch.empty((nbands, K, 4), dtype=_c64, device=coef.device) if not want_H else None
     _lib.check(_lib.load().gfdn_tf_compose_fwd(_p(turns), _p(logr), K, nbands, G, nper, _p(coef), _p(delays),
                                                _p(scale), _p(rgain), Btot // nbands, _p(direct), ldd,
-                                               _p(direct_rows), _p(filt), K, _p(H), K, _p(Ts), _p(Tq), _stream()),
+                                               _p(direct_rows), _p(filt), K, _p(H), K, _p(Ts), _p(Tq), float(dturn),
+                                               _stream()),
                "gfdn_tf_compose_fwd")
     if not want_H:
         return Tq, Ts
@@ -665,7 +667,7 @@
 
 
 def tf_compose_bwd(turns, logr, coef, delays, nper: int, rgain, gH, Tsave, filt=None, nbands: int = 1, work=None,
-                   partial: bool = False, tscale=None, gain_fold: bool = False):
+                   partial: bool = False, tscale=None, gain_fold: bool = False, dturn: float = 0.0, identity: bool = False):
     _need_gpu(turns, coef, rgain, gH, Tsave)
     if tscale is not None and (tscale.dtype != _f32 or not tscale.is_contiguous() or tscale.numel() != coef.shape[0]):
         raise RuntimeError("tf_compose_bwd: tscale must be a contiguous float32 vector with one factor per block")
@@ -675,6 +677,8 @@
     if coef.shape[0] != nbands * G or Btot % nbands or tuple(gH.shape) != (Btot, K) \
             or tuple(Tsave.shape) != (nbands * G, K):
         raise RuntimeError("tf_compose_bwd: shapes do not match nbands x G blocks")
+    if identity and Btot != nbands * G:
+        raise RuntimeError("tf_compose_bwd: identity gains need one row of gH per group")
     filt = None if filt is None else _c(filt)
     lib = _lib.load()
     if partial:
@@ -685,8 +689,9 @@
         if work is None:
             work = _work(lib.gfdn_tf_compose_bwd_work_bytes(K, nbands, G), coef.device)
     _lib.check(lib.gfdn_tf_compose_bwd(_p(turns), _p(logr), K, nbands, G, nper, _p(coef), _p(delays), _p(Tsave),
-                                       _p(tscale), _p(rgain), Btot // nbands, _p(filt), K, _p(gH), K, _p(grec), _p(work),
-                                       int(bool(gain_fold)), _stream()), "gfdn_tf_compose_bwd")
+                                       _p(tscale), None if identity else _p(rgain), Btot // nbands, _p(filt), K, _p(gH), K,
+                                       _p(grec), _p(work), int(bool(gain_fold)), float(dturn), _stream()),
+               "gfdn_tf_compose_bwd")
     return work if partial else grec
 
 
diff --git a/include/diffgfdn_hip.h b/include/diffgfdn_hip.h
--- a/include/diffgfdn_hip.h
+++ b/include/diffgfdn_hip.h
@@ -187,13 +187,13 @@
 int gfdn_tf_compose_fwd(const double* turns, const double* logr, int K, int nbands, int G, int nper,
                         const float* coef, const float* delays, const float* scale, const float* rgain, int B,
                         const float* direct_c64, int ldd, const long long* direct_rows, const float* filt_c64,
-                        int ldf, float* H_c64, int ldh, float* Tsave_c64, float* Tquad_c64, void* stream);
+                        int ldf, float* H_c64, int ldh, float* Tsave_c64, float* Tquad_c64, double dturn, void* stream);
 int gfdn_tf_compose_parts(int K);
 size_t gfdn_tf_compose_bwd_work_bytes(int K, int nbands, int G);
 int gfdn_tf_compose_bwd(const double* turns, const double* logr, int K, int nbands, int G, int nper,
                         const float* coef, const float* delays, const float* Tsave_c64, const float* tscale,
                         const float* rgain, int B, const float* filt_c64, int ldf, const float* gH_c64, int ldh,
-                        float* grec, void* work, int gain_fold, void* stream);
+                        float* grec, void* work, int gain_fold, double dturn, void* stream);
 size_t gfdn_tf_gain_grad_work_bytes(int K, int nbands, int G, int B);
 int gfdn_tf_gain_grad(int K, int nbands, int G, int B, const float* Tsave_c64, const float* filt_c64, int ldf,
                       const float* gH_c64, int ldh, float* grgain, void* work, void* stream);
```

Result: no change. 21.96 million, median of 5 (+0.7%).
